# solislemuslab/BayesianNetworkRegression.jl

Measured on NVIDIA B200. Metric: gibbs_iters_per_sec_all_chains, higher is better.
Workload: dtype f64

## Files before the change

bayesiannetworkregression.jl_b200/csrc/bnr_api.cu:

```cuda
#include <chrono>
#include <cstdio>
#include <cstdlib>
#include <cstring>
#include <mutex>
#include <string>
#include <vector>
#include <cuda_runtime.h>
#include <nvtx3/nvToolsExt.h>
#include "../../include/bnr.h"
#include "bnr_engine.cuh"
#include "bnr_kernels.h"

static_assert(BNR_ST_JITTER == BNR_ST_JITTER_ && BNR_ST_SIGMA_NOTPD == BNR_ST_SIGMA_NOTPD_ &&
              BNR_ST_G_NOTPD == BNR_ST_G_NOTPD_ && BNR_ST_GIG_CAP == BNR_ST_GIG_CAP_ &&
              BNR_ST_INJ_EXHAUSTED == BNR_ST_INJ_EXHAUSTED_ && BNR_ST_NAN == BNR_ST_NAN_ &&
              BNR_ST_PSI_NOTPD == BNR_ST_PSI_NOTPD_, "status bits out of sync");
static_assert(BNR_COND_THETA == BNR_COND_THETA_ && BNR_COND_DELTA == BNR_COND_DELTA_ && BNR_COND_M == BNR_COND_M_ &&
              BNR_COND_MU == BNR_COND_MU_ && BNR_COND_LAMBDA == BNR_COND_LAMBDA_ && BNR_COND_PI == BNR_COND_PI_,
              "conditional ids out of sync");
static_assert(BNR_MAX_R == bnr::MAX_R, "MAX_R out of sync");

using namespace bnr;

static thread_local std::string g_err;
// ... 20 lines not shown
  int c0 = 0;
  cudaStream_t stream = nullptr;
  cudaGraph_t graph[2] = {nullptr, nullptr};
  cudaGraphExec_t gexec[2] = {nullptr, nullptr};
  cudaEvent_t done = nullptr;
  ForkJoin fj;
  double* ws = nullptr;
  long long* counters = nullptr;
  long long* mom_window = nullptr;
};
constexpr int MAX_GROUPS = 8;

namespace {
struct CacheBlock { void* p; size_t bytes; int device; };
std::mutex g_cache_mu;
std::vector<CacheBlock> g_cache;
size_t g_cache_bytes = 0;
size_t g_cache_limit = (size_t)4 << 30;

void* cache_take(int device, size_t bytes, size_t* got) {
  std::lock_guard<std::mutex> lk(g_cache_mu);
  size_t best = g_cache.size();
  for (size_t i = 0; i < g_cache.size(); ++i)
    if (g_cache[i].device == device && g_cache[i].bytes >= bytes && g_cache[i].bytes <= bytes + bytes / 4 + ((size_t)1 << 20) &&
        (best == g_cache.size() || g_cache[i].bytes < g_cache[best].bytes))
      best = i;
  if (best == g_cache.size()) return nullptr;
  void* p = g_cache[best].p;
  *got = g_cache[best].bytes;
  g_cache_bytes -= g_cache[best].bytes;
  g_cache[best] = g_cache.back();
  g_cache.pop_back();
  return p;
}
void cache_give(int device, void* p, size_t bytes) {
  {
    std::lock_guard<std::mutex> lk(g_cache_mu);
    if (g_cache_bytes + bytes <= g_cache_limit) {
      g_cache.push_back({p, bytes, device});
      g_cache_bytes += bytes;
      return;
    }
  }
  cudaFree(p);
}
}

struct bnr_handle {
  bnr_params p;
  Engine e;
  cudaStream_t stream = nullptr;
  ChainGroup groups[MAX_GROUPS];
  int n_groups = 0;
  bool graphs_ready[2] = {false, false};
  const double* u_first = nullptr;
  cudaEvent_t ev_fork = nullptr;
  ForkJoin fj;
  cudaEvent_t ev0 = nullptr, ev1 = nullptr;
  std::vector<std::pair<void*, size_t>> allocs;
  double* ws = nullptr;
  double* d_inj = nullptr;
  long long inj_len = 0;
  bool aux_on = false;
  Aux aux_saved = {};
  long long win[5] = {0, 0, 0, 1, 0};
  long long blk_len = 0;
  long long mom_half = 0;
  long long launches = 0;
  long long graph_kernels = 0;
  bool xg_valid = false;
  bool ran = false;
  double* d_rhat = nullptr;
  double* d_tmp = nullptr;
  size_t tmp_doubles = 0;
  double* d_acov = nullptr;
  double* d_cmean = nullptr;
  int ess_lag = -1;
  long long ess_rows = 0;
  size_t acov_cap = 0;
  long long* d_esswin = nullptr;
  double* ess_stream_buf = nullptr;
  size_t ess_stream_cap = 0;
  long long ess_stream_N = 0;
};

static int raw_alloc(bnr_handle* h, void** out, size_t bytes) {
  size_t got = bytes;
  void* p = cache_take(h->p.device, bytes, &got);
  if (!p) { CK(cudaMalloc(&p, bytes)); got = bytes; }
  h->allocs.push_back({p, got});
  *out = p;
  return 0;
}

static void release_alloc(bnr_handle* h, void* p) {
  if (!p) return;
  for (size_t i = 0; i < h->allocs.size(); ++i)
    if (h->allocs[i].first == p) {
      cache_give(h->p.device, p, h->allocs[i].second);
      h->allocs[i] = h->allocs.back();
      h->allocs.pop_back();
      return;
    }
}

struct Scratch {
  int device; void* p = nullptr; size_t bytes = 0;
  Scratch(int dev, size_t b) : device(dev), bytes((b + 255) / 256 * 256) {
    size_t got = bytes;
    p = cache_take(device, bytes, &got);
    if (p) bytes = got;
    else if (cudaMalloc(&p, bytes) != cudaSuccess) p = nullptr;
  }
  ~Scratch() { if (p) cache_give(device, p, bytes); }
};

template <typename T>
static int dalloc(bnr_handle* h, T** ptr, size_t count, bool zero = true) {
  void* p = nullptr;
  const size_t bytes = count * sizeof(T) + 16;
  int r = raw_alloc(h, &p, bytes);
  if (r) return r;
  if (zero) CK(cudaMemsetAsync(p, 0, bytes, h->stream));
  *ptr = (T*)p;
  return 0;
}
static int alloc_table(bnr_handle* h, RowTable& t, bool nan_fill, const char* what) {
  if (int r = dalloc(h, &t.base, t.doubles(), false)) {
    cudaGetLastError();
    return fail(r, std::string(what) + " (" + std::to_string(8.0 * (double)t.doubles()) + " bytes): " + g_err);
  }
  if (nan_fill) CK(cudaMemsetAsync(t.base, 0xff, sizeof(double) * t.doubles(), h->stream));
  return BNR_OK;
}
#define DA(ptr, count)                          \
  do {                                          \
    int _r = dalloc(h, &(ptr), (count));        \
    if (_r) return _r;                          \
  } while (0)

extern "C" int bnr_version(void) { return BNR_VERSION; }
extern "C" const char* bnr_last_error(void) { return g_err.c_str(); }

extern "C" void bnr_default_params(bnr_params* p) {
  memset(p, 0, sizeof(*p));
  p->num_chains = 2;
  p->eta = 1.01; p->zeta = 1.0; p->iota = 1.0; p->a_delta = 1.0; p->b_delta = 1.0; p->nu = 10.0;
  p->trace_full_chains = 1; p->trace_gamma_xi_all = 1; p->gig_inject_len = 64;
}

static int var_size(const Dims& d, int var) {
  switch (var) {
    case BNR_VAR_TAU2: case BNR_VAR_THETA: case BNR_VAR_DELTA: case BNR_VAR_MU: return 1;
    case BNR_VAR_U: return d.R * d.V;
    case BNR_VAR_XI: return d.V;
    case BNR_VAR_GAMMA: case BNR_VAR_S: return d.q;
    case BNR_VAR_M: return d.R * d.R;
    case BNR_VAR_LAMBDA: return d.R;
    case BNR_VAR_PI: return 3 * d.R;
  }
  return -1;
}
static int row_offset(const Dims& d, int var) {
  const int R = d.R, V = d.V, q = d.q;
  const int o[BNR_NUM_VARS] = {0, 1, 1 + V * R, 1 + V * R + V, 1 + V * R + V + q, 1 + V * R + V + 2 * q,
                               2 + V * R + V + 2 * q, 3 + V * R + V + 2 * q, 3 + V * R + V + 2 * q + R * R,
                               4 + V * R + V + 2 * q + R * R, 4 + V * R + V + 2 * q + R * R + R};
  return o[var];
}

static int create_fork_join(ForkJoin& f, int panels, int side_prio, int hi_prio) {
  CK(cudaStreamCreateWithPriority(&f.side, cudaStreamNonBlocking, side_prio));
  CK(cudaStreamCreateWithPriority(&f.side_hi, cudaStreamNonBlocking, hi_prio));
  CK(cudaEventCreateWithFlags(&f.fork, cudaEventDisableTiming));
  CK(cudaEventCreateWithFlags(&f.join, cudaEventDisableTiming));
  f.npool = 4 * panels;
  f.pool = new cudaEvent_t[f.npool]();
  for (int i = 0; i < f.npool; ++i) CK(cudaEventCreateWithFlags(&f.pool[i], cudaEventDisableTiming));
  return BNR_OK;
}

static void destroy_fork_join(ForkJoin& f) {
  if (f.side) cudaStreamDestroy(f.side);
  if (f.side_hi) cudaStreamDestroy(f.side_hi);
  if (f.fork) cudaEventDestroy(f.fork);
  if (f.join) cudaEventDestroy(f.join);
  for (int i = 0; i < f.npool && f.pool; ++i)
    if (f.pool[i]) cudaEventDestroy(f.pool[i]);
  delete[] f.pool;
  f = ForkJoin();
}

static int create_impl(bnr_handle* h, const bnr_params* p, const double* X, const double* y);

extern "C" int bnr_create(const bnr_params* p, const double* X, const double* y, bnr_handle** out) {
  if (!p || !X || !y || !out) return fail(BNR_EINVAL, "null argument");
  if (p->n < 1 || p->V < 2 || p->R < 1 || p->R > BNR_MAX_R || p->num_chains < 1)
    return fail(BNR_EINVAL, "need n >= 1, V >= 2, 1 <= R <= 16, num_chains >= 1");
  if (!(p->nu > p->R - 1)) return fail(BNR_EINVAL, "nu must exceed R - 1 (InverseWishart degrees of freedom)");
  int ndev = 0;
  if (cudaGetDeviceCount(&ndev) != cudaSuccess || ndev == 0)
    return fail(BNR_ENODEV, "no CUDA device visible: libbnr has no CPU fallback");
  if (p->device < 0 || p->device >= ndev) return fail(BNR_EINVAL, "device ordinal out of range");
  CK(cudaSetDevice(p->device));
  int cc_major = 0;
  CK(cudaDeviceGetAttribute(&cc_major, cudaDevAttrComputeCapabilityMajor, p->device));
  if (cc_major < 10) return fail(BNR_ENODEV, "libbnr is built for sm_100a (B200) only");

  bnr_handle* h = new bnr_handle();
  h->p = *p;
  const double t0 = wall_ms();
  const int rc = create_impl(h, p, X, y);
  if (g_timing) fprintf(stderr, "[bnr] bnr_create %.2f ms (%zu device buffers)\n", wall_ms() - t0, h->allocs.size());
  if (rc != BNR_OK) {
    const std::string msg = g_err;
    bnr_destroy(h);
    g_err = msg;
    return rc;
  }
  *out = h;
  return BNR_OK;
}

static int create_impl(bnr_handle* h, const bnr_params* p, const double* X, const double* y) {
  if (h->p.gig_inject_len <= 0) h->p.gig_inject_len = 64;
  Dims& d = h->e.d;
  d.n = p->n; d.V = p->V; d.R = p->R; d.C = p->num_chains; d.C_total = p->num_chains;
  d.q = p->V * (p->V + 1) / 2;
  d.np = (p->n + 1 + TILE_N - 1) / TILE_N * TILE_N;
  d.qp = (d.q + TILE_K - 1) / TILE_K * TILE_K;
  {
    const double qd = d.q, nd = d.n;
    const double cost_q = qd * qd * qd / 3.0 + 4.0 * qd * qd, cost_n = nd * nd * qd + nd * nd * nd / 3.0;
    const int qp128 = (d.q + 1 + TILE_N - 1) / TILE_N * TILE_N;
    const int small = bwd_stream_max_dim(), large = chol_max_dim();
    int mode = p->gamma_mode;
    if (mode != BNR_GAMMA_NFORM && mode != BNR_GAMMA_QFORM) {
      mode = (cost_q < cost_n && qp128 <= small) ? BNR_GAMMA_QFORM : BNR_GAMMA_NFORM;
      if ((mode == BNR_GAMMA_QFORM ? qp128 : d.np) > small) {
        const bool q_fits = qp128 <= large, n_fits = d.np <= large;
        mode = (q_fits && (cost_q < cost_n || !n_fits)) ? BNR_GAMMA_QFORM : BNR_GAMMA_NFORM;
      }
    }
    d.gmode = mode;
    if (mode == BNR_GAMMA_QFORM) d.qp = qp128;
    d.gdim = mode == BNR_GAMMA_QFORM ? d.qp : d.np;
  }
  d.nparts = (d.q + PART_BLOCK - 1) / PART_BLOCK;
  d.chain_offset = p->chain_offset;
  d.chain_offset_local = 0;
  d.gigK = h->p.gig_inject_len;
  d.seed = p->seed;
  d.eta = p->eta; d.zeta = p->zeta; d.iota = p->iota; d.a_delta = p->a_delta; d.b_delta = p->b_delta; d.nu = p->nu;
  const size_t need = sizeof(double) * ((size_t)d.V * d.R + 2 * d.R * d.R + 2 + 4 * (2 * d.V + 2 * d.R * d.R + 3 * d.R));
  if (need > 200 * 1024 || d.gdim > chol_max_dim()) {
    return fail(BNR_EINVAL, "problem too large for the per-chain shared-memory kernels (V*R > 200 KB of shared memory, or factored dimension > 32768: n <= 32767 in the n-form, V <= 255 in the q-form)");
  }
  CK(cudaStreamCreateWithFlags(&h->stream, cudaStreamNonBlocking));
  CK(cudaEventCreate(&h->ev0));
  CK(cudaEventCreate(&h->ev1));
  linalg_setup();
  {
    const int clusters = bwd_cluster_capacity(d.gdim);
    if (clusters < 0) return fail(BNR_ECUDA, "cudaOccupancyMaxActiveClusters failed for the cluster back solve");
    if (clusters == 0)
      return fail(BNR_ECUDA, "this device cannot co-schedule the back solve's cluster of 8 CTAs with ~210 KB of shared memory each (factored dimension > 8192)");
  }
  if (!tmap_setup()) return fail(BNR_ECUDA, "cuTensorMapEncodeTiled is not available from this driver (TMA tensor maps are required)");
  small_kernels_setup();

  Engine& e = h->e;
  const size_t C = d.C;
  const double t_create0 = wall_ms();
  double *dX, *dy;
  DA(dX, (size_t)d.qp * d.np);
  DA(dy, (size_t)d.np);
  CK(cudaMemcpy2DAsync(dX, (size_t)d.np * sizeof(double), X, (size_t)d.n * sizeof(double),
                       (size_t)d.n * sizeof(double), (size_t)d.q, cudaMemcpyHostToDevice, h->stream));
  CK(cudaMemcpyAsync(dy, y, (size_t)d.n * sizeof(double), cudaMemcpyHostToDevice, h->stream));
  e.X = dX; e.y = dy;
  if (g_timing) { cudaStreamSynchronize(h->stream); fprintf(stderr, "[bnr]   X, y upload done at +%.2f ms\n", wall_ms() - t_create0); }
  std::vector<int2> lk(d.q);
  {
    int j = 0;
    for (int k = 0; k < d.V; ++k)
      for (int l = k; l < d.V; ++l) lk[j++] = make_int2(l, k);
  }
  int2* dlk;
  DA(dlk, (size_t)d.q);
  CK(cudaMemcpyAsync(dlk, lk.data(), sizeof(int2) * d.q, cudaMemcpyHostToDevice, h->stream));
  CK(cudaStreamSynchronize(h->stream));
  e.edge_lk = dlk;

  DA(e.tau2, C); DA(e.u, C * d.V * d.R); DA(e.u_alt, C * d.V * d.R); DA(e.xi, C * d.V);
  h->u_first = e.u;
  DA(e.gamma, C * d.qp); DA(e.S, C * d.qp); DA(e.theta, C); DA(e.Delta, C); DA(e.M, C * d.R * d.R);
  DA(e.mu, C); DA(e.lambda, C * d.R); DA(e.pi, C * 3 * d.R);
  DA(e.W, C * d.qp); DA(e.v, C * d.qp); DA(e.t, C * d.qp);
  DA(e.xg, C * d.np); DA(e.xv, C * d.np); DA(e.rhs, C * d.np);
  DA(e.G, C * d.gdim * d.gdim + 2048);
  DA(e.Linv, C * (size_t)(d.gdim / TILE_N) * TILE_N * TILE_N);
  CK(cudaMemsetAsync(e.Linv, 0, sizeof(double) * C * (size_t)(d.gdim / TILE_N) * TILE_N * TILE_N, h->stream));
  e.syrk_ws = nullptr; e.syrk_ws_cap = 0;
  e.gram_planes = nullptr; e.gram_rscale = nullptr;
  if (gram_i8_selected(d)) {
    DA(e.gram_planes, C * gram_i8_plane_bytes(d));
    DA(e.gram_rscale, C * d.np);
  } else if (d.gmode == BNR_GAMMA_NFORM) {
    const int smax = syrk_splits(d, d.C);
    if (smax > 1) {
      e.syrk_ws_cap = smax - 1;
      DA(e.syrk_ws, C * (size_t)e.syrk_ws_cap * d.gdim * d.gdim);
    }
  }
  e.XtX = nullptr;
  if (d.gmode == BNR_GAMMA_QFORM) {
    std::vector<double> xt((size_t)d.np * d.qp, 0.0), ones((size_t)d.np, 1.0);
    for (int j = 0; j < d.q; ++j)
      for (int i = 0; i < d.n; ++i) xt[(size_t)i * d.qp + j] = X[(size_t)i + (size_t)d.n * j];
    double *dXT = nullptr, *dOnes = nullptr, *dXtX = nullptr;
    DA(dXT, xt.size());
    DA(dOnes, ones.size());
    DA(dXtX, (size_t)d.qp * d.qp);
    CK(cudaMemcpyAsync(dXT, xt.data(), xt.size() * sizeof(double), cudaMemcpyHostToDevice, h->stream));
    CK(cudaMemcpyAsync(dOnes, ones.data(), ones.size() * sizeof(double), cudaMemcpyHostToDevice, h->stream));
    launch_xtx(d, dXT, dOnes, dXtX, h->stream);
    CK(cudaStreamSynchronize(h->stream));
    release_alloc(h, dXT);
    release_alloc(h, dOnes);
    e.XtX = dXtX;
  }
  DA(e.partials, C * d.nparts * (2 * MAX_R + 1));
  DA(e.tau2_part, C * 2 * TAU2_MAX_BLOCKS);
  DA(e.tau2_ticket, C);
  DA(e.status, C);
  DA(e.iter, 1); DA(e.trace_row, 1);
  DA(e.moments, C * 2 * (d.V + d.q) * 2);
  DA(e.mom_window, 5);
  e.bmom = nullptr; e.bmom_nb = 0;
  e.ess_ring = e.ess_head = e.ess_acc = e.ess_sum = nullptr; e.ess_win = nullptr; e.ess_L = e.ess_cap = 0;
  DA(h->d_esswin, 4);
  DA(h->ws, x_times_workspace_doubles(d));
  DA(h->d_rhat, (size_t)(d.V + d.q));
  const long long trace_rows = p->trace_rows > 0 ? p->trace_rows : 0;
  e.tr_full = {nullptr, trace_rows, 4 + d.V * d.R + d.V + 2 * d.q + d.R * d.R + d.R + 3 * d.R, 0};
  e.tr_gx = {nullptr, trace_rows, d.V + d.q, 0};
  if (trace_rows > 0) {
    e.tr_full.chains = p->trace_full_chains < 0 ? 0 : (p->trace_full_chains < d.C ? p->trace_full_chains : d.C);
    if (p->trace_gamma_xi_all) e.tr_gx.chains = d.C;
    else if (p->trace_gamma_xi_chains > 0) e.tr_gx.chains = p->trace_gamma_xi_chains < d.C ? p->trace_gamma_xi_chains : d.C;
  }
  if (e.tr_full.chains > 0) if (int r = alloc_table(h, e.tr_full, false, "full-state trace")) return r;
  if (e.tr_gx.chains > 0) if (int r = alloc_table(h, e.tr_gx, false, "gamma/xi trace")) return r;
  {
    int ng_auto = d.C >= 6 ? 3 : (d.C >= 4 ? 4 : (d.C >= 2 ? 2 : 1));
    if (d.gmode == BNR_GAMMA_NFORM && d.C >= 4 && syrk_splits(d, d.C) > 1) ng_auto = 2;
    if (d.gmode == BNR_GAMMA_QFORM && d.C >= 2 && d.C < 24) ng_auto = 2;
    if (gram_i8_selected(d) && d.C < 12) ng_auto = 1;
    int ng = p->chain_groups > 0 ? p->chain_groups : ng_auto;
    if (ng > MAX_GROUPS) ng = MAX_GROUPS;
    if (ng > d.C) ng = d.C;
    h->n_groups = ng;
    CK(cudaEventCreateWithFlags(&h->ev_fork, cudaEventDisableTiming));
    const int panels = d.gdim / TILE_N;
    if (int r = create_fork_join(h->fj, panels, 0, 0)) return r;
    int plo = 0, phi = 0;
    CK(cudaDeviceGetStreamPriorityRange(&plo, &phi));
    for (int g = 0; g < ng; ++g) {
      ChainGroup& G = h->groups[g];
      CK(cudaStreamCreateWithPriority(&G.stream, cudaStreamNonBlocking, phi));
      CK(cudaEventCreateWithFlags(&G.done, cudaEventDisableTiming));
      if (int r = create_fork_join(G.fj, panels, plo, phi)) return r;
      DA(G.ws, x_times_workspace_doubles(d));
      DA(G.counters, 2);
      DA(G.mom_window, 5);
    }
  }
  if (g_timing) { cudaStreamSynchronize(h->stream); fprintf(stderr, "[bnr]   buffers, streams, events at +%.2f ms\n", wall_ms() - t_create0); }
  h->tmp_doubles = (size_t)1 << 22;
  DA(h->d_tmp, h->tmp_doubles);
  e.inj = nullptr; e.inj_stride = 0;
  memset(&e.aux, 0, sizeof(e.aux));
  CK(cudaStreamSynchronize(h->stream));
  if (!tmaps_check(e)) return fail(BNR_ECUDA, "cuTensorMapEncodeTiled refused a tensor map of this problem's geometry");
  return BNR_OK;
}

static void drop_graph(bnr_handle* h);

extern "C" int bnr_trim_cache(void) {
  std::vector<CacheBlock> blocks;
  {
    std::lock_guard<std::mutex> lk(g_cache_mu);
    blocks.swap(g_cache);
    g_cache_bytes = 0;
  }
  int cur = 0;
  cudaGetDevice(&cur);
  for (auto& b : blocks) { cudaSetDevice(b.device); cudaFree(b.p); }
  cudaSetDevice(cur);
  return BNR_OK;
}

extern "C" int bnr_set_cache_limit(int64_t bytes) {
  if (bytes < 0) return fail(BNR_EINVAL, "negative limit");
  { std::lock_guard<std::mutex> lk(g_cache_mu); g_cache_limit = (size_t)bytes; }
  if (bytes == 0) return bnr_trim_cache();
  return BNR_OK;
}

extern "C" int bnr_destroy(bnr_handle* h) {
  if (!h) return BNR_OK;
  const double t_destroy0 = wall_ms();
  cudaSetDevice(h->p.device);
  if (h->stream) cudaStreamSynchronize(h->stream);
  drop_graph(h);
  for (int g = 0; g < h->n_groups; ++g) {
    if (h->groups[g].stream) { cudaStreamSynchronize(h->groups[g].stream); cudaStreamDestroy(h->groups[g].stream); }
    if (h->groups[g].done) cudaEventDestroy(h->groups[g].done);
    destroy_fork_join(h->groups[g].fj);
  }
  destroy_fork_join(h->fj);
  if (h->ev_fork) cudaEventDestroy(h->ev_fork);
  for (auto& a : h->allocs) cache_give(h->p.device, a.first, a.second);
  if (h->ev0) cudaEventDestroy(h->ev0);
  if (h->ev1) cudaEventDestroy(h->ev1);
  if (h->stream) cudaStreamDestroy(h->stream);
  delete h;
  if (g_timing) fprintf(stderr, "[bnr] bnr_destroy %.2f ms\n", wall_ms() - t_destroy0);
  return BNR_OK;
}

static void drop_graph(bnr_handle* h) {
  for (int g = 0; g < h->n_groups; ++g) {
    ChainGroup& G = h->groups[g];
    for (int par = 0; par < 2; ++par) {
      if (G.gexec[par]) { cudaGraphExecDestroy(G.gexec[par]); G.gexec[par] = nullptr; }
      if (G.graph[par]) { cudaGraphDestroy(G.graph[par]); G.graph[par] = nullptr; }
    }
  }
  h->graphs_ready[0] = h->graphs_ready[1] = false;
}

static void refresh_xg(bnr_handle* h) {
  launch_x_times(h->e, 0, h->e.gamma, h->e.xg, h->ws, h->stream);
  h->xg_valid = true;
}

static void mark(cudaEvent_t* marks, int k, cudaStream_t s) {
  if (marks) cudaEventRecord(marks[k], s);
}

static void run_gamma(Engine& e, double* ws, const ForkJoin& fj, cudaStream_t s, int gig_flags, bool syrk_forked = false,
                      cudaEvent_t* marks = nullptr) {
  if (e.d.gmode == BNR_GAMMA_QFORM) {
    launch_edge_prep(e, 2, s);
    launch_x_times(e, 0, e.W, e.xv, ws, s);
    launch_rhs(e, s);
    launch_x_times(e, 1, e.rhs, e.t, ws, s);
    mark(marks, 3, s);
    launch_build_P(e, s);
    mark(marks, 4, s);
    launch_cholesky(e, e.t, fj, s);
    mark(marks, 5, s);
    launch_chol_solve(e, e.t, e.v, s);
    mark(marks, 6, s);
    launch_gamma_gig(e, (gig_flags & ~1) | ((gig_flags & 1) ? 4 : 0), s);
    return;
  }
  launch_edge_prep(e, 1, s);
  launch_x_times(e, 0, e.v, e.xv, ws, s);
  launch_rhs(e, s);
  mark(marks, 3, s);
  if (syrk_forked) cudaStreamWaitEvent(s, fj.join, 0);
  else launch_syrk_G(e, s);
  mark(marks, 4, s);
  launch_cholesky(e, e.rhs, fj, s);
  mark(marks, 5, s);
  launch_chol_solve(e, e.rhs, nullptr, s);
  mark(marks, 6, s);
  launch_x_times(e, 1, e.rhs, e.t, ws, s);
  launch_gamma_gig(e, gig_flags, s);
}

static void enqueue_record(Engine& e, double* ws, const ForkJoin& fj, cudaStream_t s, bool sweep_done, bool pred_forked,
                           bool xg_stale) {
  launch_record(e, sweep_done, s);
  if (sweep_done && e.ess_ring) launch_ess_stream(e, s);
  if (e.pred.base) {
    if (pred_forked) cudaStreamWaitEvent(s, fj.join, 0);
    else launch_pred_product(e, s);
    launch_pred_record(e, sweep_done, s);
  }
  if (e.ll.base) {
    if (xg_stale) launch_x_times(e, 0, e.gamma, e.xg, ws, s);
    launch_loglik_record(e, s);
  }
  launch_advance(e, sweep_done, s);
}

static void enqueue_sweep(Engine& e, double* ws, const ForkJoin& fj, cudaStream_t s, cudaEvent_t* marks = nullptr) {
  NvtxRange sweep("bnr sweep");
  mark(marks, 0, s);
  const bool fork_syrk = !marks && e.d.gmode == BNR_GAMMA_NFORM && !e.aux.G_copy;
  if (fork_syrk) {
    NvtxRange r("gamma: G = X D X' + I (forked)");
    cudaEventRecord(fj.fork, s);
    cudaStreamWaitEvent(fj.side, fj.fork, 0);
    launch_syrk_G(e, fj.side);
    cudaEventRecord(fj.join, fj.side);
  }
  { NvtxRange r("tau2"); launch_tau2(e, s); }
  mark(marks, 1, s);
  { NvtxRange r("u, xi"); launch_uxi(e, s); }
  std::swap(e.u, e.u_alt);
  mark(marks, 2, s);
  { NvtxRange r("gamma + D (GIG)"); run_gamma(e, ws, fj, s, 3, fork_syrk, marks); }
  mark(marks, 7, s);
  const bool fork_pred = !marks && e.pred.base;
  if (fork_pred) {
    NvtxRange r("predictions: X_new gamma");
    cudaEventRecord(fj.fork, s);
    cudaStreamWaitEvent(fj.side, fj.fork, 0);
    launch_pred_product(e, fj.side);
    cudaEventRecord(fj.join, fj.side);
  }
  {
    NvtxRange r("theta, Delta, M, mu, Lambda, pi");
    launch_x_times(e, 0, e.gamma, e.xg, ws, s);
    launch_finish(e, (1 << BNR_COND_THETA) | (1 << BNR_COND_DELTA) | (1 << BNR_COND_M) | (1 << BNR_COND_MU) |
                         (1 << BNR_COND_LAMBDA) | (1 << BNR_COND_PI), s);
  }
  NvtxRange r("record");
  enqueue_record(e, ws, fj, s, true, fork_pred, false);
  mark(marks, 8, s);
}

static Engine group_view(const bnr_handle* h, int c0, int Cg, long long* counters, long long* mom_window) {
  Engine v = h->e;
  const Dims& d = h->e.d;
  const size_t c = (size_t)c0;
  v.d.C = Cg;
  v.d.chain_offset = d.chain_offset + c0;
  v.d.chain_offset_local = c0;
  v.tau2 += c; v.theta += c; v.Delta += c; v.mu += c; v.status += c;
  v.u += c * d.V * d.R; v.u_alt += c * d.V * d.R; v.xi += c * d.V;
  v.gamma += c * d.qp; v.S += c * d.qp; v.W += c * d.qp; v.v += c * d.qp; v.t += c * d.qp;
  v.M += c * d.R * d.R; v.lambda += c * d.R; v.pi += c * 3 * d.R;
  v.xg += c * d.np; v.xv += c * d.np; v.rhs += c * d.np;
  v.G += c * d.gdim * d.gdim; if (v.syrk_ws) v.syrk_ws += c * (size_t)v.syrk_ws_cap * d.gdim * d.gdim; v.Linv += c * (size_t)(d.gdim / TILE_N) * TILE_N * TILE_N;
  if (v.gram_planes) { v.gram_planes += c * gram_i8_plane_bytes(d); v.gram_rscale += c * d.np; }
  v.partials += c * d.nparts * (2 * MAX_R + 1);
  v.moments += c * 2 * (d.V + d.q) * 2;
  if (v.bmom) v.bmom += c * (size_t)v.bmom_nb * (d.V + d.q) * 2;
  if (v.ess_ring) {
    const size_t P = (size_t)d.V + d.q;
    v.ess_ring += c * (size_t)v.ess_cap * P; v.ess_head += c * (size_t)v.ess_L * P;
    v.ess_acc += c * (size_t)(v.ess_L + 1) * P; v.ess_sum += c * 2 * P;
  }
  v.tr_full = v.tr_full.view(c0, Cg); v.tr_gx = v.tr_gx.view(c0, Cg);
  v.pred = v.pred.view(c0, Cg); v.ll = v.ll.view(c0, Cg);
  if (v.pred_ws) v.pred_ws += c * (size_t)v.pred_splits * v.pred_mp;
  v.iter = counters; v.trace_row = counters + 1; v.mom_window = mom_window;
  v.inj = nullptr; v.inj_stride = 0;
  memset(&v.aux, 0, sizeof(v.aux));
  return v;
}

static int build_graphs(bnr_handle* h) {
  const int par = (h->e.u != h->u_first) ? 1 : 0;
  if (h->graphs_ready[par]) return BNR_OK;
  const double t0 = wall_ms();
  const long long before = g_launches;
  const int C = h->e.d.C, ng = h->n_groups;
  for (int g = 0; g < ng; ++g) {
    ChainGroup& G = h->groups[g];
    const int c0 = (int)((long long)C * g / ng), c1 = (int)((long long)C * (g + 1) / ng);
    G.c0 = c0;
    G.e = group_view(h, c0, c1 - c0, G.counters, G.mom_window);
    Engine e = G.e;
    CK(cudaStreamBeginCapture(G.stream, cudaStreamCaptureModeThreadLocal));
    enqueue_sweep(e, G.ws, G.fj, G.stream);
    enqueue_sweep(e, G.ws, G.fj, G.stream);
    CK(cudaStreamEndCapture(G.stream, &G.graph[par]));
    CK(cudaGraphInstantiate(&G.gexec[par], G.graph[par], cudaGraphInstantiateFlagUseNodePriority));
  }
  h->graph_kernels = g_launches - before;
  h->graphs_ready[par] = true;
  if (g_timing) fprintf(stderr, "[bnr] graph capture + instantiate (%d groups, %lld kernels) %.2f ms\n", ng, h->graph_kernels, wall_ms() - t0);
  return BNR_OK;
}

extern "C" int bnr_init_state(bnr_handle* h) {
  if (!h) return fail(BNR_EINVAL, "null handle");
  CK(cudaSetDevice(h->p.device));
  Engine& e = h->e;
  CK(cudaMemsetAsync(e.iter, 0, sizeof(long long), h->stream));
  CK(cudaMemsetAsync(e.trace_row, 0, sizeof(long long), h->stream));
  CK(cudaMemsetAsync(e.status, 0, sizeof(int) * e.d.C, h->stream));
  launch_init(e, h->stream);
  enqueue_record(e, h->ws, h->fj, h->stream, false, false, true);
  h->xg_valid = false;
  CK(cudaGetLastError());
  CK(cudaStreamSynchronize(h->stream));
  return BNR_OK;
}

extern "C" int bnr_run(bnr_handle* h, int64_t n_iters) {
  if (!h || n_iters < 0) return fail(BNR_EINVAL, "bad arguments");
  NvtxRange range("bnr_run");
  CK(cudaSetDevice(h->p.device));
  CK(cudaEventRecord(h->ev0, h->stream));
  if (!h->xg_valid) { const long long b0 = g_launches; refresh_xg(h); h->launches += g_launches - b0; }
  int64_t left = n_iters;
  if (h->e.inj == nullptr && !h->aux_on && left >= 2) {
    int r = build_graphs(h);
    if (r) return r;
    const int par = (h->e.u != h->u_first) ? 1 : 0;
    CK(cudaEventRecord(h->ev_fork, h->stream));
    for (int g = 0; g < h->n_groups; ++g) {
      ChainGroup& G = h->groups[g];
      CK(cudaStreamWaitEvent(G.stream, h->ev_fork, 0));
      CK(cudaMemcpyAsync(G.counters, h->e.iter, sizeof(long long), cudaMemcpyDeviceToDevice, G.stream));
      CK(cudaMemcpyAsync(G.counters + 1, h->e.trace_row, sizeof(long long), cudaMemcpyDeviceToDevice, G.stream));
    }
    for (; left >= 2; left -= 2) {
      for (int g = 0; g < h->n_groups; ++g) CK(cudaGraphLaunch(h->groups[g].gexec[par], h->groups[g].stream));
      h->launches += h->graph_kernels;
    }
    for (int g = 0; g < h->n_groups; ++g) {
      CK(cudaEventRecord(h->groups[g].done, h->groups[g].stream));
      CK(cudaStreamWaitEvent(h->stream, h->groups[g].done, 0));
    }
    CK(cudaMemcpyAsync(h->e.iter, h->groups[0].counters, sizeof(long long), cudaMemcpyDeviceToDevice, h->stream));
    CK(cudaMemcpyAsync(h->e.trace_row, h->groups[0].counters + 1, sizeof(long long), cudaMemcpyDeviceToDevice, h->stream));
  }
  for (; left > 0; --left) {
    const long long before = g_launches;
    enqueue_sweep(h->e, h->ws, h->fj, h->stream);
    h->launches += g_launches - before;
  }
  CK(cudaEventRecord(h->ev1, h->stream));
  if (h->e.inj == nullptr && !h->aux_on && (h->graphs_ready[0] || h->graphs_ready[1])) {
    int r = build_graphs(h);
    if (r) return r;
  }
  CK(cudaGetLastError());
  h->ran = true;
  return BNR_OK;
}

extern "C" int bnr_sync(bnr_handle* h) {
  if (!h) return fail(BNR_EINVAL, "null handle");
  CK(cudaSetDevice(h->p.device));
  CK(cudaStreamSynchronize(h->stream));
  CK(cudaGetLastError());
  return BNR_OK;
}

extern "C" int bnr_last_run_ms(bnr_handle* h, float* ms) {
  if (!h || !ms || !h->ran) return fail(BNR_ESTATE, "no run recorded");
  CK(cudaSetDevice(h->p.device));
  CK(cudaEventSynchronize(h->ev1));
  CK(cudaEventElapsedTime(ms, h->ev0, h->ev1));
  return BNR_OK;
}

extern "C" int bnr_iteration(bnr_handle* h, int64_t* completed) {
  if (!h || !completed) return fail(BNR_EINVAL, "null argument");
  CK(cudaSetDevice(h->p.device));
  long long v = 0;
  CK(cudaMemcpyAsync(&v, h->e.iter, sizeof(v), cudaMemcpyDeviceToHost, h->stream));
  CK(cudaStreamSynchronize(h->stream));
  *completed = v;
  return BNR_OK;
}

extern "C" int bnr_set_trace_row(bnr_handle* h, int64_t row) {
  if (!h || row < 0) return fail(BNR_EINVAL, "bad arguments");
  CK(cudaSetDevice(h->p.device));
  long long v = row;
  CK(cudaMemcpyAsync(h->e.trace_row, &v, sizeof(v), cudaMemcpyHostToDevice, h->stream));
  CK(cudaStreamSynchronize(h->stream));
  return BNR_OK;
}

extern "C" int bnr_get_trace_row(bnr_handle* h, int64_t* row) {
  if (!h || !row) return fail(BNR_EINVAL, "null argument");
  CK(cudaSetDevice(h->p.device));
  long long v = 0;
  CK(cudaMemcpyAsync(&v, h->e.trace_row, sizeof(v), cudaMemcpyDeviceToHost, h->stream));
  CK(cudaStreamSynchronize(h->stream));
  *row = v;
  return BNR_OK;
}

extern "C" int bnr_copy_trace_rows(bnr_handle* h, int64_t dst, int64_t src, int64_t count) {
  if (!h || dst < 0 || src < 0 || count < 0) return fail(BNR_EINVAL, "bad arguments");
  CK(cudaSetDevice(h->p.device));
  Engine& e = h->e;
  const struct { const RowTable& t; const char* range_msg; } all[] = {
      {e.tr_full, "rows out of range"}, {e.tr_gx, "rows out of range"},
      {e.pred, "rows beyond the prediction table"}, {e.ll, "rows beyond the log-likelihood table"}};
  bool any = false;
  int max_row = 0;
  for (const auto& a : all) {
    if (!a.t.base) continue;
    if (dst + count > a.t.rows || src + count > a.t.rows) return fail(BNR_EINVAL, a.range_msg);
    if (a.t.width > max_row) max_row = a.t.width;
    any = true;
  }
  if (!any) return BNR_OK;
  if (count == 0 || dst == src) return BNR_OK;
  const bool overlap = !(dst + count <= src || src + count <= dst);
  Scratch sc(h->p.device, overlap ? (size_t)count * max_row * sizeof(double) : 256);
  if (overlap && !sc.p) return fail(BNR_ENOMEM, "device scratch allocation failed");
  for (const auto& a : all) {
    if (!a.t.base) continue;
    const size_t bytes = (size_t)count * a.t.width * sizeof(double);
    for (int c = 0; c < a.t.chains; ++c) {
      if (!overlap) {
        CK(cudaMemcpyAsync(a.t.row(c, dst), a.t.row(c, src), bytes, cudaMemcpyDeviceToDevice, h->stream));
      } else {
        CK(cudaMemcpyAsync(sc.p, a.t.row(c, src), bytes, cudaMemcpyDeviceToDevice, h->stream));
        CK(cudaMemcpyAsync(a.t.row(c, dst), sc.p, bytes, cudaMemcpyDeviceToDevice, h->stream));
      }
    }
  }
  CK(cudaStreamSynchronize(h->stream));
  return BNR_OK;
}

static int push_windows(bnr_handle* h) {
  CK(cudaMemcpyAsync(h->e.mom_window, h->win, sizeof(h->win), cudaMemcpyHostToDevice, h->stream));
  for (int g = 0; g < h->n_groups; ++g)
    CK(cudaMemcpyAsync(h->groups[g].mom_window, h->win, sizeof(h->win), cudaMemcpyHostToDevice, h->stream));
  CK(cudaStreamSynchronize(h->stream));
  return BNR_OK;
}

extern "C" int bnr_set_moment_window(bnr_handle* h, int64_t first, int64_t len) {
  if (!h || len < 0) return fail(BNR_EINVAL, "bad arguments");
  CK(cudaSetDevice(h->p.device));
  h->win[0] = first; h->win[1] = len;
  int r = push_windows(h);
  if (r) return r;
  h->mom_half = len / 2;
  return BNR_OK;
}

extern "C" int bnr_set_moment_blocks(bnr_handle* h, int64_t first_sweep, int64_t block_len, int32_t nblocks) {
  if (!h || nblocks < 0 || (nblocks > 0 && block_len < 1)) return fail(BNR_EINVAL, "bad arguments");
  CK(cudaSetDevice(h->p.device));
  const Dims& d = h->e.d;
  if (nblocks > h->e.bmom_nb) {
    CK(cudaStreamSynchronize(h->stream));
    drop_graph(h);
    void* p = nullptr;
    release_alloc(h, h->e.bmom);
    h->e.bmom = nullptr; h->e.bmom_nb = 0;
    int r = raw_alloc(h, &p, sizeof(double) * (size_t)d.C * nblocks * (d.V + d.q) * 2);
    if (r) return r;
    h->e.bmom = (double*)p;
    h->e.bmom_nb = nblocks;
  }
  h->win[2] = first_sweep; h->win[3] = block_len > 0 ? block_len : 1; h->win[4] = nblocks;
  h->blk_len = block_len;
  return push_windows(h);
}

__global__ void k_merge_blocks(const double* __restrict__ bmom, int nb_cap, int nparam, int first_block, int per_half,
                               long long blen, double* __restrict__ mom) {
  const int p = blockIdx.x * blockDim.x + threadIdx.x;
  if (p >= nparam) return;
  const int c = blockIdx.y, half = blockIdx.z;
  double n = 0.0, mean = 0.0, m2 = 0.0;
  for (int b = 0; b < per_half; ++b) {
    const double* m = bmom + (((size_t)c * nb_cap + first_block + half * per_half + b) * nparam + p) * 2;
    const double nb_ = (double)blen, delta = m[0] - mean, tot = n + nb_;
    mean += delta * nb_ / tot;
    m2 += m[1] + delta * delta * n * nb_ / tot;
    n = tot;
  }
  double* o = mom + (((size_t)c * 2 + half) * nparam + p) * 2;
  o[0] = mean; o[1] = m2;
}

extern "C" int bnr_moments_from_blocks(bnr_handle* h, int32_t first_block, int32_t nblocks) {
  if (!h || first_block < 0 || nblocks < 2 || (nblocks & 1)) return fail(BNR_EINVAL, "need an even number of blocks >= 2");
  CK(cudaSetDevice(h->p.device));
  if (!h->e.bmom || first_block + nblocks > (int)h->win[4]) return fail(BNR_ESTATE, "blocks not configured (bnr_set_moment_blocks)");
  const Dims& d = h->e.d;
  const int np_ = d.V + d.q;
  dim3 grid((np_ + 127) / 128, d.C, 2);
  k_merge_blocks<<<grid, 128, 0, h->stream>>>(h->e.bmom, h->e.bmom_nb, np_, first_block, nblocks / 2, h->blk_len, h->e.moments);
  CK(cudaGetLastError());
  CK(cudaStreamSynchronize(h->stream));
  h->mom_half = (long long)(nblocks / 2) * h->blk_len;
  return BNR_OK;
}

extern "C" int bnr_moments_device(bnr_handle* h, double** dev_ptr, int64_t* count) {
  if (!h || !dev_ptr || !count) return fail(BNR_EINVAL, "null argument");
  CK(cudaSetDevice(h->p.device));
  CK(cudaStreamSynchronize(h->stream));
  *dev_ptr = h->e.moments;
  *count = (int64_t)h->e.d.C * 2 * (h->e.d.V + h->e.d.q) * 2;
  return BNR_OK;
}

extern "C" int bnr_rhat_from_moments(int device, const double* dev_moments, int32_t total_chains, int32_t V,
                                     int32_t q, int64_t half_len, double* rhat_xi, double* rhat_gamma) {
  if (!dev_moments || total_chains < 1 || half_len < 2) return fail(BNR_EINVAL, "bad arguments (need half_len >= 2)");
  CK(cudaSetDevice(device));
  Scratch sc(device, sizeof(double) * (V + q));
  if (!sc.p) return fail(BNR_ENOMEM, "device scratch allocation failed");
  double* d_out = (double*)sc.p;
  launch_rhat(dev_moments, total_chains, V + q, half_len, d_out, 0);
  std::vector<double> host(V + q);
  CK(cudaMemcpy(host.data(), d_out, sizeof(double) * (V + q), cudaMemcpyDeviceToHost));
  if (rhat_xi) memcpy(rhat_xi, host.data(), sizeof(double) * V);
  if (rhat_gamma) memcpy(rhat_gamma, host.data() + V, sizeof(double) * q);
  return BNR_OK;
}

__global__ void k_moments_from_trace(RowTable tr, long long first, long long nrows, double* __restrict__ mom) {
  const int nparam = tr.width, p = blockIdx.x * blockDim.x + threadIdx.x;
  if (p >= nparam) return;
  const int c = blockIdx.y, half = blockIdx.z;
  const long long h = nrows / 2;
  const long long r0 = first + (half == 0 ? 0 : nrows - h);
  const double* __restrict__ base = tr.row(c, r0) + p;
  double s = 0.0;
  for (long long r = 0; r < h; ++r) s += base[(size_t)r * nparam];
  const double mean = s / (double)h;
  double m2 = 0.0;
  for (long long r = 0; r < h; ++r) { const double dl = base[(size_t)r * nparam] - mean; m2 += dl * dl; }
  double* m = mom + (((size_t)c * 2 + half) * nparam + p) * 2;
  m[0] = mean; m[1] = m2;
}

extern "C" int bnr_moments_from_trace(bnr_handle* h, int64_t first_row, int64_t nrows) {
  if (!h || first_row < 0 || nrows < 0) return fail(BNR_EINVAL, "bad arguments");
  CK(cudaSetDevice(h->p.device));
  Engine& e = h->e;
  if (!e.tr_gx.base || e.tr_gx.chains < e.d.C)
    return fail(BNR_ESTATE, "gamma/xi traces of every chain are needed (trace_gamma_xi_all = 0): use the streaming "
                            "moments of bnr_set_moment_window instead");
  if (first_row + nrows > e.tr_gx.rows) return fail(BNR_EINVAL, "rows beyond trace capacity");
  if (nrows / 2 < 2) return fail(BNR_EINVAL, "need at least 4 rows");
  dim3 grid((e.tr_gx.width + 127) / 128, e.d.C, 2);
  k_moments_from_trace<<<grid, 128, 0, h->stream>>>(e.tr_gx, first_row, nrows, e.moments);
  CK(cudaGetLastError());
  CK(cudaStreamSynchronize(h->stream));
  h->mom_half = nrows / 2;
  return BNR_OK;
}

extern "C" int bnr_moment_half_len(bnr_handle* h, int64_t* half_len) {
  if (!h || !half_len) return fail(BNR_EINVAL, "null argument");
  CK(cudaSetDevice(h->p.device));
  *half_len = h->mom_half;
  return BNR_OK;
}

extern "C" int bnr_rhat(bnr_handle* h, double* rhat_xi, double* rhat_gamma) {
  if (!h) return fail(BNR_EINVAL, "null handle");
  CK(cudaSetDevice(h->p.device));
  if (h->mom_half < 2) return fail(BNR_ESTATE, "moment window too short for R-hat");
  const Dims& d = h->e.d;
  launch_rhat(h->e.moments, d.C, d.V + d.q, h->mom_half, h->d_rhat, h->stream);
  std::vector<double> host(d.V + d.q);
  CK(cudaMemcpyAsync(host.data(), h->d_rhat, sizeof(double) * (d.V + d.q), cudaMemcpyDeviceToHost, h->stream));
  CK(cudaStreamSynchronize(h->stream));
  if (rhat_xi) memcpy(rhat_xi, host.data(), sizeof(double) * d.V);
  if (rhat_gamma) memcpy(rhat_gamma, host.data() + d.V, sizeof(double) * d.q);
  return BNR_OK;
}

extern "C" int bnr_var_size(bnr_handle* h, int32_t var, int64_t* n) {
  if (!h || !n || var < 0 || var >= BNR_NUM_VARS) return fail(BNR_EINVAL, "bad arguments");
  CK(cudaSetDevice(h->p.device));
// ... 738 lines not shown
```

bayesiannetworkregression.jl_b200/csrc/bnr_engine.cuh:

```cuda
#pragma once
#include <cstdint>
#include <cuda_runtime.h>
#include "bnr_rng.cuh"

namespace bnr {

constexpr int MAX_R = 16;
constexpr int TILE_N = 128;
constexpr int TILE_K = 16;
constexpr int TAU2_MAX_BLOCKS = 32;
constexpr int PART_BLOCK = 256;

struct Dims {
  int n, V, R, q, C;
  int C_total;
  int np, qp;
  int gmode;
  int gdim;
  int nparts;
  int chain_offset;
  int chain_offset_local;
  int gigK;
  uint64_t seed;
  double eta, zeta, iota, a_delta, b_delta, nu;
};

struct InjLayout {
  int64_t tau2, uxi, z1, z2, S, theta, Delta, M, mu, lambda, pi, total;
  __host__ __device__ static InjLayout make(int n, int V, int R, int K) {
    InjLayout l;
    const int64_t q = (int64_t)V * (V + 1) / 2;
    int64_t o = 0;
    l.tau2 = o; o += 1;
    l.uxi = o; o += (int64_t)V * (R + 1);
    l.z1 = o; o += q;
    l.z2 = o; o += n;
    l.S = o; o += q * K;
    l.theta = o; o += 1;
    l.Delta = o; o += 3;
    l.M = o; o += R + R * (R - 1) / 2;
    l.mu = o; o += 1;
    l.lambda = o; o += R;
    l.pi = o; o += 3 * R;
    l.total = o;
    return l;
  }
};

struct InitLayout {
  int64_t S, pi, lambda, xi, M, u, gamma, total;
  __host__ __device__ static InitLayout make(int V, int R) {
    InitLayout l;
    const int64_t q = (int64_t)V * (V + 1) / 2;
    int64_t o = 0;
    l.S = o; o += q;
    l.pi = o; o += 3 * R;
    l.lambda = o; o += R;
    l.xi = o; o += V;
    l.M = o; o += R + R * (R - 1) / 2;
    l.u = o; o += (int64_t)V * R;
    l.gamma = o; o += q;
    l.total = o;
    return l;
  }
};

struct Aux {
  double* tau2_params;
  double* sigma_inv;
  double* sigma_chol;
  double* mu_t;
  double* log_odds;
  double* chi;
  double* theta_params;
  double* delta_params;
  double* m_params;
  double* mu_params;
  double* lambda_logw;
  double* lambda_w;
  double* pi_alpha;
  double* gig_used;
  double* G_copy;
};

struct RowTable {
  double* base; long long rows; int width; int chains;
  __host__ __device__ bool holds(int c, long long r) const { return base && c < chains && r < rows; }
  __host__ __device__ double* row(int c, long long r) const { return base + ((size_t)c * rows + r) * width; }
  RowTable view(int c0, int Cg) const {
    RowTable v = *this;
    v.chains = chains - c0 < 0 ? 0 : (chains - c0 > Cg ? Cg : chains - c0);
    v.base = base && v.chains > 0 ? row(c0, 0) : nullptr;
    return v;
  }
  size_t doubles() const { return (size_t)chains * rows * width; }
};

struct Engine {
  Dims d;
  const double* X;
  const double* y;
  const int2* edge_lk;
  const double* XtX;
  double* tau2; double* u; double* u_alt; double* xi; double* gamma; double* S; double* theta;
  double* Delta; double* M; double* mu; double* lambda; double* pi;
  double* W;
  double* v;
  double* t;
  double* xg;
  double* xv;
  double* rhs;
  double* G;
  double* syrk_ws;
  int syrk_ws_cap;
  signed char* gram_planes;
  double* gram_rscale;
  double* Linv;
  double* partials;
  double* tau2_part;
  unsigned* tau2_ticket;
  int* status;
  long long* iter;
  long long* trace_row;
  double* moments;
  long long* mom_window;
  double* bmom;
  int bmom_nb;
  double* ess_ring;
  double* ess_head;
  double* ess_acc;
  double* ess_sum;
  const long long* ess_win;
  int ess_L, ess_cap;
  RowTable tr_full;
  RowTable tr_gx;
  RowTable pred;
  const double* Xp;
  int pred_mp, pred_mode, pred_splits;
  double* pred_ws;
  RowTable ll;
  const double* inj;
  long long inj_stride;
  Aux aux;
};

__device__ __forceinline__ RngKey chain_key(const Dims& d, int c) {
  return make_key(d.seed, (uint32_t)(d.chain_offset + c));
}

}
```

bayesiannetworkregression.jl_b200/csrc/bnr_kernels.h:

```cpp
#pragma once
#include <cuda_runtime.h>
#include "bnr_engine.cuh"

#define BNR_ST_JITTER_ 1
#define BNR_ST_SIGMA_NOTPD_ 2
#define BNR_ST_G_NOTPD_ 4
#define BNR_ST_GIG_CAP_ 8
#define BNR_ST_INJ_EXHAUSTED_ 16
#define BNR_ST_NAN_ 32
#define BNR_ST_PSI_NOTPD_ 64
#define BNR_COND_THETA_ 4
#define BNR_COND_DELTA_ 5
#define BNR_COND_M_ 6
#define BNR_COND_MU_ 7
#define BNR_COND_LAMBDA_ 8
#define BNR_COND_PI_ 9

namespace bnr {

extern thread_local long long g_launches;

void launch_tau2(const Engine& e, cudaStream_t s);
void launch_uxi(const Engine& e, cudaStream_t s);
void launch_edge_prep(const Engine& e, int draw_v, cudaStream_t s);
void launch_rhs(const Engine& e, cudaStream_t s);
void launch_gamma_gig(const Engine& e, int flags, cudaStream_t s);
void launch_finish(const Engine& e, int mask, cudaStream_t s);
void launch_init(const Engine& e, cudaStream_t s);
void launch_record(const Engine& e, int sweep_done, cudaStream_t s);
void launch_advance(const Engine& e, int inc_iter, cudaStream_t s);
void launch_rhat(const double* mom, int chains, int nparams, long long h, double* out, cudaStream_t s);
void launch_test_chol_jitter(int R, const double* Ain, double* Aused, double* Lout, int* status, cudaStream_t s);
void launch_rng_dump(const Dims& d, int chain, long long iteration, int site, int element, int kind, double shape,
                     int count, double* out, cudaStream_t s);

void launch_x_times(const Engine& e, int trans, const double* in, double* out, double* splitk_ws, cudaStream_t s);
void launch_x_times(const Dims& d, int trans, const double* A, int lda, int M, int K, const double* in, double* out,
                    double* splitk_ws, cudaStream_t s);
size_t x_times_workspace_doubles(const Dims& d);
int pred_splits(const Dims& d, int mp);
void launch_pred_product(const Engine& e, cudaStream_t s);
void launch_pred_record(const Engine& e, int sweep_done, cudaStream_t s);
void launch_loglik_record(const Engine& e, cudaStream_t s);
void launch_syrk_G(const Engine& e, cudaStream_t s);
int syrk_splits(const Dims& d, int C);
constexpr int GRAM_I8_QP_MIN = 1024;
constexpr int GRAM_I8_QP_MAX = 18724;
bool gram_i8_selected(const Dims& d);
size_t gram_i8_plane_bytes(const Dims& d);
struct ForkJoin {
  cudaStream_t side = nullptr;
  cudaStream_t side_hi = nullptr;
  cudaEvent_t fork = nullptr, join = nullptr;
  cudaEvent_t* pool = nullptr;
  int npool = 0;
};
void launch_cholesky(const Engine& e, double* rhs, const ForkJoin& fj, cudaStream_t s);
void launch_chol_solve(const Engine& e, double* rhs, const double* addz, cudaStream_t s);
void launch_xtx(const Dims& d, const double* XT, const double* ones, double* XtX, cudaStream_t s);
void launch_build_P(const Engine& e, cudaStream_t s);
int chol_max_dim();
int bwd_stream_max_dim();
int bwd_cluster_capacity(int N);
bool tmaps_check(const Engine& e);
bool tmap_setup();
void linalg_setup();
void small_kernels_setup();

void launch_summary_select(const double* rows, size_t rowlen, int off, int nelem, long long first, long long count,
                           long long rank_lo, long long rank_hi, double* mean_out, double* lo_out, double* hi_out,
                           cudaStream_t s);
void launch_chain_mean(const RowTable& tr, long long first, long long N, double* cmean, cudaStream_t s);
void launch_acov_sum(const RowTable& tr, long long first, long long N, int L, const double* cmean, double* acov,
                     cudaStream_t s);
void launch_ess_stream(const Engine& e, cudaStream_t s);
void launch_ess_stream_finalize(const Engine& e, long long N, double* acov, double* cmean, cudaStream_t s);
size_t pred_select_ws_bytes(long long N, int m);
void launch_pred_select(const double* rows, long long N, int m, long long rank_lo, long long rank_hi, double* mean,
                        double* lo, double* hi, void* ws, cudaStream_t s);
long long loo_tail_len(long long N);
long long loo_tail_max();
size_t loo_ws_bytes(long long N, int n);
void launch_loo(const double* rows, long long N, int n, double* out, void* ws, cudaStream_t s);
void launch_ess_finish(const double* acov_parts, int nparts, const double* cmeans, int chains, int P, long long N,
                       int L, double* ess, double* lag_used, cudaStream_t s);

}
```

bayesiannetworkregression.jl_b200/csrc/bnr_linalg.cu:

```cuda
#include <cstdio>
#include <cstdlib>
#include <cstring>
#include <cuda.h>
#include "bnr_engine.cuh"
#include "bnr_kernels.h"

namespace bnr {

__device__ __forceinline__ void dmma884(double& c0, double& c1, double a, double b) {
  asm volatile("mma.sync.aligned.m8n8k4.row.col.f64.f64.f64.f64 {%0,%1}, {%2}, {%3}, {%0,%1};\n"
               : "+d"(c0), "+d"(c1) : "d"(a), "d"(b));
}
__device__ __forceinline__ double neg_bits(double x) {
  return __longlong_as_double(__double_as_longlong(x) ^ (long long)0x8000000000000000ull);
}
__device__ __forceinline__ void cp_async_commit() { asm volatile("cp.async.commit_group;\n" ::); }
template <int N>
__device__ __forceinline__ void cp_async_wait() { asm volatile("cp.async.wait_group %0;\n" ::"n"(N)); }
__device__ __forceinline__ void cp_async16(void* smem, const void* gmem) {
  const unsigned sa = (unsigned)__cvta_generic_to_shared(smem);
  asm volatile("cp.async.cg.shared.global [%0], [%1], 16;\n" ::"r"(sa), "l"(gmem));
}

__device__ __forceinline__ unsigned smem_u32(const void* p) { return (unsigned)__cvta_generic_to_shared(p); }
// ... 1070 lines not shown
    for (int s = 0; s < nstages; ++s) { mbar_init(&full[s], 1); mbar_init(&empty[s], 8); }
    for (int s = 0; s < BWC_SLOTS; ++s) mbar_init(&sfull[s], 8 * (BWC_K - 1));
    for (int i = 0; i < BWC_K * BWC_SLOTS; ++i) mbar_init(&sfree[i], 1);
    asm volatile("fence.mbarrier_init.release.cluster;\n" ::: "memory");
  }
  __syncthreads();
  cluster_sync_all();

  if (warp == 8) {
    if (lane == 0) {
      int p = 0;
      for (int J = T - 1; J >= 0; --J) {
        const int Ilast = (J % BWC_K == r) ? J : J + 1;
        for (int I = Itop; I >= Ilast; I -= BWC_K) {
          for (int h = 0; h < BW_NH; ++h, ++p) {
            const int stage = p % nstages;
            mbar_wait(&empty[stage], ((p / nstages) & 1) ^ 1);
            mbar_expect_tx(&full[stage], BW_STAGE_DBL * 8u);
            double* dst = ring + (size_t)stage * BW_STAGE_DBL;
            if (I == J) tma_load_2d(dst, &tmL, 0, (c * T + J) * PB + h * BW_COLS, &full[stage]);
            else tma_load_2d(dst, &tmG, I * PB, c * N + J * PB + h * BW_COLS, &full[stage]);
          }
        }
      }
    }
  } else {
    const double unscale = out[(size_t)c * out_stride + m];
    for (int id = tid; id < nown * PB; id += 256) {
      const int I = r + BWC_K * (id / PB), k = I * PB + id % PB;
      xo[id] = (I < T && k < m) ? Gc[(size_t)k * N + m] * unscale + (addz ? addz[(size_t)c * addz_stride + k] : 0.0) : 0.0;
    }
    named_bar_sync(1, 256);

    int it = 0;
    for (int J = T - 1; J >= 0; --J) {
      const int o = J % BWC_K, u = (T - 1 - J) / BWC_K;
      const int s = u % BWC_SLOTS;
      const unsigned par = (u / BWC_SLOTS) & 1;
      double pr[BW_NH][BW_CPW];
#pragma unroll
      for (int h = 0; h < BW_NH; ++h)
#pragma unroll
        for (int q = 0; q < BW_CPW; ++q) pr[h][q] = 0.0;
      for (int I = Itop; I > J; I -= BWC_K) {
        const double* v = xo + (size_t)(I / BWC_K) * PB;
        const double v0 = v[lane], v1 = v[lane + 32], v2 = v[lane + 64], v3 = v[lane + 96];
#pragma unroll
        for (int h = 0; h < BW_NH; ++h, ++it) {
          const int stage = it % nstages;
          mbar_wait(&full[stage], (it / nstages) & 1);
          const double* B = ring + (size_t)stage * BW_STAGE_DBL + (size_t)(warp * BW_CPW) * PB + lane;
          double acc[BW_CPW];
#pragma unroll
          for (int q = 0; q < BW_CPW; ++q)
            acc[q] = B[q * PB] * v0 + B[q * PB + 32] * v1 + B[q * PB + 64] * v2 + B[q * PB + 96] * v3;
#pragma unroll
          for (int q = 0; q < BW_CPW; ++q) {
#pragma unroll
            for (int o2 = 16; o2 > 0; o2 >>= 1) acc[q] += __shfl_xor_sync(0xffffffffu, acc[q], o2);
            pr[h][q] += acc[q];
          }
          __syncwarp();
          if (lane == 0) mbar_arrive(&empty[stage]);
        }
      }
      if (o != r) {
        if (lane == 0) {
          mbar_wait_cluster(&sfree[o * BWC_SLOTS + s], par ^ 1);
          const unsigned dst = mapa_rank(slot + ((size_t)s * BWC_K + r) * PB, (unsigned)o);
#pragma unroll
          for (int h = 0; h < BW_NH; ++h)
#pragma unroll
            for (int q = 0; q < BW_CPW; ++q) st_cluster_f64(dst + 8u * (h * BW_COLS + warp * BW_CPW + q), pr[h][q]);
          mbar_arrive_remote(mapa_rank(&sfull[s], (unsigned)o));
        }
        __syncwarp();
        continue;
      }
      double* bJ = xo + (size_t)(J / BWC_K) * PB;
      if (lane == 0) {
        mbar_wait_cluster(&sfull[s], par);
        const double* sl = slot + (size_t)s * BWC_K * PB;
#pragma unroll
        for (int h = 0; h < BW_NH; ++h)
#pragma unroll
          for (int q = 0; q < BW_CPW; ++q) {
            const int col = h * BW_COLS + warp * BW_CPW + q;
            double t = bJ[col];
#pragma unroll
            for (int rr = 0; rr < BWC_K; ++rr) t -= (rr == r) ? pr[h][q] : sl[rr * PB + col];
            bJ[col] = t;
          }
      }
      __syncwarp();
      named_bar_sync(1, 256);
      if (tid == 0) {
        for (int rr = 0; rr < BWC_K; ++rr)
          if (rr != r) mbar_arrive_remote(mapa_rank(&sfree[r * BWC_SLOTS + s], (unsigned)rr));
      }
      const double v0 = bJ[lane], v1 = bJ[lane + 32], v2 = bJ[lane + 64], v3 = bJ[lane + 96];
      double xn[BW_NH][BW_CPW];
#pragma unroll
      for (int h = 0; h < BW_NH; ++h, ++it) {
        const int stage = it % nstages;
        mbar_wait(&full[stage], (it / nstages) & 1);
        const double* B = ring + (size_t)stage * BW_STAGE_DBL + (size_t)(warp * BW_CPW) * PB + lane;
        double acc[BW_CPW];
#pragma unroll
        for (int q = 0; q < BW_CPW; ++q)
          acc[q] = B[q * PB] * v0 + B[q * PB + 32] * v1 + B[q * PB + 64] * v2 + B[q * PB + 96] * v3;
#pragma unroll
        for (int q = 0; q < BW_CPW; ++q) {
#pragma unroll
          for (int o2 = 16; o2 > 0; o2 >>= 1) acc[q] += __shfl_xor_sync(0xffffffffu, acc[q], o2);
          xn[h][q] = acc[q];
        }
        __syncwarp();
        if (lane == 0) mbar_arrive(&empty[stage]);
      }
      named_bar_sync(1, 256);
      if (lane == 0) {
#pragma unroll
        for (int h = 0; h < BW_NH; ++h)
#pragma unroll
          for (int q = 0; q < BW_CPW; ++q) bJ[h * BW_COLS + warp * BW_CPW + q] = xn[h][q];
      }
      __syncwarp();
      named_bar_sync(1, 256);
    }
    for (int id = tid; id < nown * PB; id += 256) {
      const int I = r + BWC_K * (id / PB);
      if (I < T) out[(size_t)c * out_stride + (size_t)I * PB + id % PB] = xo[id];
    }
  }
  cluster_sync_all();
}

__global__ void k_copy_sym(const double* __restrict__ G, size_t chain_stride, int np, double* __restrict__ out) {
  const int c = blockIdx.y, j = blockIdx.x;
  const double* Gc = G + (size_t)c * chain_stride;
  double* o = out + (size_t)c * np * np;
  for (int i = threadIdx.x; i < np; i += blockDim.x) {
    const double v = (i >= j) ? Gc[(size_t)j * np + i] : Gc[(size_t)i * np + j];
    o[(size_t)j * np + i] = v;
  }
}

constexpr int XM_BM = 128, XM_BN = 64, XM_BK = 16, XM_STAGES = 3;
constexpr int XM_LDM = 132, XM_LDK = 20;
constexpr int XM_A_DBL = (XM_BK * XM_LDM > XM_BM * XM_LDK) ? XM_BK * XM_LDM : XM_BM * XM_LDK;
constexpr int XM_STAGE_DBL = XM_A_DBL + XM_BN * XM_LDK;
constexpr size_t XMMA_SMEM = sizeof(double) * XM_STAGES * XM_STAGE_DBL;

__device__ __forceinline__ void cp_async16_zfill(void* smem, const void* gmem, bool valid) {
  const unsigned sa = (unsigned)__cvta_generic_to_shared(smem);
  const int sz = valid ? 16 : 0;
  asm volatile("cp.async.cg.shared.global [%0], [%1], 16, %2;\n" ::"r"(sa), "l"(gmem), "r"(sz));
}

template <int TRANS>
__global__ void __launch_bounds__(256) k_xmma(const double* __restrict__ X, int np, int M, int K, int N,
                                              const double* __restrict__ in, int ldin, double* __restrict__ out,
                                              int ldout, int k_per_split) {
  extern __shared__ __align__(16) double sm[];
  const int tid = threadIdx.x, lane = tid & 31, warp = tid >> 5;
  const int lk = lane & 3, lr = lane >> 2, wm = warp & 3, wn = warp >> 2;
  const int m0 = blockIdx.x * XM_BM, n0 = blockIdx.y * XM_BN;
  const int kbeg = blockIdx.z * k_per_split;
  const int kend = min(K, kbeg + k_per_split);
  const int nsteps = (kend - kbeg + XM_BK - 1) / XM_BK;
  double* o = out + (size_t)blockIdx.z * N * ldout;

  auto load_stage = [&](int step) {
    double* As = sm + (size_t)(step % XM_STAGES) * XM_STAGE_DBL;
    double* Vs = As + XM_A_DBL;
    const int k0 = kbeg + step * XM_BK;
    if (TRANS == 0) {
#pragma unroll
      for (int r = 0; r < 4; ++r) {
        const int id = tid + 256 * r, kk = id >> 6, mm = (id & 63) * 2;
        cp_async16_zfill(As + kk * XM_LDM + mm, X + (size_t)(k0 + kk) * np + m0 + mm, m0 + mm < M);
      }
    } else {
#pragma unroll
      for (int r = 0; r < 4; ++r) {
        const int id = tid + 256 * r, mm = id >> 3, kk = (id & 7) * 2;
        const bool ok = m0 + mm < M;
        cp_async16_zfill(As + mm * XM_LDK + kk, X + (size_t)(ok ? m0 + mm : 0) * np + k0 + kk, ok);
      }
    }
#pragma unroll
    for (int r = 0; r < 2; ++r) {
      const int id = tid + 256 * r, nn = id >> 3, kk = (id & 7) * 2;
      const bool ok = n0 + nn < N;
      cp_async16_zfill(Vs + nn * XM_LDK + kk, in + (size_t)(ok ? n0 + nn : 0) * ldin + k0 + kk, ok);
    }
  };

  double acc[4][4][2];
#pragma unroll
  for (int a = 0; a < 4; ++a)
#pragma unroll
    for (int b = 0; b < 4; ++b) acc[a][b][0] = acc[a][b][1] = 0.0;
  int nfv = (N - n0 - wn * 32 + 7) >> 3;
  nfv = nfv < 0 ? 0 : (nfv > 4 ? 4 : nfv);

  for (int s = 0; s < XM_STAGES - 1; ++s) {
    if (s < nsteps) load_stage(s);
    cp_async_commit();
  }
  for (int step = 0; step < nsteps; ++step) {
    cp_async_wait<XM_STAGES - 2>();
    __syncthreads();
    if (step + XM_STAGES - 1 < nsteps) load_stage(step + XM_STAGES - 1);
    cp_async_commit();
    const double* As = sm + (size_t)(step % XM_STAGES) * XM_STAGE_DBL;
    const double* Vs = As + XM_A_DBL;
    if (nfv == 0) continue;
#pragma unroll
    for (int k4 = 0; k4 < XM_BK / 4; ++k4) {
      const int kr = k4 * 4 + lk;
      double af[4], bf[4];
#pragma unroll
      for (int mf = 0; mf < 4; ++mf)
        af[mf] = (TRANS == 0) ? As[kr * XM_LDM + wm * 32 + mf * 8 + lr] : As[(wm * 32 + mf * 8 + lr) * XM_LDK + kr];
#pragma unroll
      for (int nf = 0; nf < 4; ++nf) bf[nf] = (nf < nfv) ? Vs[(wn * 32 + nf * 8 + lr) * XM_LDK + kr] : 0.0;
#pragma unroll
      for (int nf = 0; nf < 4; ++nf) {
        if (nf < nfv) {
#pragma unroll
          for (int mf = 0; mf < 4; ++mf) dmma884(acc[mf][nf][0], acc[mf][nf][1], af[mf], bf[nf]);
        }
      }
    }
  }
  cp_async_wait<0>();
#pragma unroll
  for (int mf = 0; mf < 4; ++mf) {
    const int mm = m0 + wm * 32 + mf * 8 + lr;
#pragma unroll
    for (int nf = 0; nf < 4; ++nf) {
      const int nn = n0 + wn * 32 + nf * 8 + 2 * lk;
      if (mm < M) {
        if (nn < N) o[(size_t)nn * ldout + mm] = acc[mf][nf][0];
        if (nn + 1 < N) o[(size_t)(nn + 1) * ldout + mm] = acc[mf][nf][1];
      }
    }
  }
}

__global__ void k_splitk_reduce(const double* __restrict__ ws, double* __restrict__ out, size_t count, int splits) {
  const size_t i = (size_t)blockIdx.x * blockDim.x + threadIdx.x;
  if (i >= count) return;
  double s = 0.0;
  for (int z = 0; z < splits; ++z) s += ws[(size_t)z * count + i];
  out[i] = s;
}

static int x_times_splits(int M, int K, int C_total) {
  const int tiles = ((M + XM_BM - 1) / XM_BM) * ((C_total + XM_BN - 1) / XM_BN);
  int ks = (2 * 148 + tiles - 1) / tiles;
  const int kmax = K / (4 * XM_BK) > 0 ? K / (4 * XM_BK) : 1;
  if (ks > kmax) ks = kmax;
  if (ks > 64) ks = 64;
  if (ks < 1) ks = 1;
  return ks;
}

size_t x_times_workspace_doubles(const Dims& d) {
  const int a = x_times_splits(d.np, d.qp, d.C_total), b = x_times_splits(d.qp, d.np, d.C_total);
  const size_t wa = (size_t)a * d.C_total * d.np, wb = (size_t)b * d.C_total * d.qp;
  return wa > wb ? wa : wb;
}

int pred_splits(const Dims& d, int mp) { return x_times_splits(mp, d.qp, d.C_total); }

void launch_x_times(const Dims& d, int trans, const double* A, int lda, int M, int K, const double* in, double* out,
                    double* ws, cudaStream_t s) {
  const int N = d.C, ldin = K, ldout = M;
  const int ks = x_times_splits(M, K, d.C_total);
  const int kper = ((K + ks - 1) / ks + XM_BK - 1) / XM_BK * XM_BK;
  dim3 grid((M + XM_BM - 1) / XM_BM, (N + XM_BN - 1) / XM_BN, ks);
  double* dst = (ks == 1 && out) ? out : ws;
  ++g_launches;
  if (trans) k_xmma<1><<<grid, 256, XMMA_SMEM, s>>>(A, lda, M, K, N, in, ldin, dst, ldout, kper);
  else k_xmma<0><<<grid, 256, XMMA_SMEM, s>>>(A, lda, M, K, N, in, ldin, dst, ldout, kper);
  if (ks > 1 && out) {
    const size_t count = (size_t)N * ldout;
    ++g_launches; k_splitk_reduce<<<(unsigned)((count + 255) / 256), 256, 0, s>>>(ws, out, count, ks);
  }
}

void launch_x_times(const Engine& e, int trans, const double* in, double* out, double* ws, cudaStream_t s) {
  const Dims& d = e.d;
  launch_x_times(d, trans, e.X, d.np, trans ? d.qp : d.np, trans ? d.np : d.qp, in, out, ws, s);
}

void launch_pred_product(const Engine& e, cudaStream_t s) {
  launch_x_times(e.d, 0, e.Xp, e.pred_mp, e.pred_mp, e.d.qp, e.gamma, nullptr, e.pred_ws, s);
}

__global__ void k_gram_i8(const __grid_constant__ CUtensorMap tmA, const __grid_constant__ CUtensorMap tmB,
                          const double* __restrict__ rscale, double* __restrict__ G, int np, int nvalid, int nkb);
extern const size_t GI_SMEM_BYTES;

void linalg_setup() {
  cudaFuncSetAttribute(k_xmma<0>, cudaFuncAttributeMaxDynamicSharedMemorySize, (int)XMMA_SMEM);
  cudaFuncSetAttribute(k_xmma<1>, cudaFuncAttributeMaxDynamicSharedMemorySize, (int)XMMA_SMEM);
  cudaFuncSetAttribute(k_gram_syrk, cudaFuncAttributeMaxDynamicSharedMemorySize, (int)SYRK_SMEM);
  cudaFuncSetAttribute(k_gram_i8, cudaFuncAttributeMaxDynamicSharedMemorySize, (int)GI_SMEM_BYTES);
  cudaFuncSetAttribute(k_chol_update, cudaFuncAttributeMaxDynamicSharedMemorySize, (int)SYRK_SMEM);
  cudaFuncSetAttribute(k_trsm_dmma, cudaFuncAttributeMaxDynamicSharedMemorySize, (int)SYRK_SMEM);
  cudaFuncSetAttribute(k_potf2_inv, cudaFuncAttributeMaxDynamicSharedMemorySize, (int)POTF2_SMEM);
  cudaFuncSetAttribute(k_bwd_stream, cudaFuncAttributeMaxDynamicSharedMemorySize, 227 * 1024);
  cudaFuncSetAttribute(k_bwd_cluster, cudaFuncAttributeMaxDynamicSharedMemorySize, 227 * 1024);
  cudaFuncSetAttribute(k_small_tile<1, 4>, cudaFuncAttributeMaxDynamicSharedMemorySize, (int)small_tile_smem(32));
  cudaFuncSetAttribute(k_small_tile<2, 4>, cudaFuncAttributeMaxDynamicSharedMemorySize, (int)small_tile_smem(32));
  cudaFuncSetAttribute(k_small_tile<1, 2>, cudaFuncAttributeMaxDynamicSharedMemorySize, (int)small_tile_smem(16));
  cudaFuncSetAttribute(k_small_tile<2, 2>, cudaFuncAttributeMaxDynamicSharedMemorySize, (int)small_tile_smem(16));
  cudaFuncSetAttribute(k_small_tile<1, 8>, cudaFuncAttributeMaxDynamicSharedMemorySize, (int)small_tile_smem(64));
  cudaFuncSetAttribute(k_small_tile<2, 8>, cudaFuncAttributeMaxDynamicSharedMemorySize, (int)small_tile_smem(64));
}

typedef CUresult (*TmapEncodeFn)(CUtensorMap*, CUtensorMapDataType, cuuint32_t, void*, const cuuint64_t*, const cuuint64_t*,
                                 const cuuint32_t*, const cuuint32_t*, CUtensorMapInterleave, CUtensorMapSwizzle,
                                 CUtensorMapL2promotion, CUtensorMapFloatOOBfill);
static TmapEncodeFn g_tmap_encode = nullptr;
bool tmap_setup() {
  if (g_tmap_encode) return true;
  void* fn = nullptr;
  cudaDriverEntryPointQueryResult qr;
  if (cudaGetDriverEntryPoint("cuTensorMapEncodeTiled", &fn, cudaEnableDefault, &qr) != cudaSuccess ||
      qr != cudaDriverEntryPointSuccess || !fn)
    return false;
  g_tmap_encode = (TmapEncodeFn)fn;
  return true;
}
static CUresult encode_map(CUtensorMap* m, const double* base, uint64_t rows, uint64_t krows, uint64_t ld, uint32_t box_rows,
                           uint32_t box_k) {
  memset(m, 0, sizeof(*m));
  const cuuint64_t dims[2] = {rows, krows};
  const cuuint64_t strides[1] = {ld * sizeof(double)};
  const cuuint32_t box[2] = {box_rows, box_k};
  const cuuint32_t estr[2] = {1, 1};
  if (!tmap_setup()) return CUDA_ERROR_NOT_SUPPORTED;
  return g_tmap_encode(m, CU_TENSOR_MAP_DATA_TYPE_FLOAT64, 2, const_cast<double*>(base), dims, strides, box, estr,
                       CU_TENSOR_MAP_INTERLEAVE_NONE, CU_TENSOR_MAP_SWIZZLE_NONE, CU_TENSOR_MAP_L2_PROMOTION_L2_256B,
                       CU_TENSOR_MAP_FLOAT_OOB_FILL_NONE);
}
static CUtensorMap make_map(const double* base, uint64_t rows, uint64_t krows, uint64_t ld, uint32_t box_rows,
                            uint32_t box_k = SY_BK) {
  CUtensorMap m;
  const CUresult r = encode_map(&m, base, rows, krows, ld, box_rows, box_k);
  if (r != CUDA_SUCCESS) {
    fprintf(stderr, "[bnr] cuTensorMapEncodeTiled failed (%d) for a %llu x %llu operand, box %u x %d\n", (int)r,
            (unsigned long long)rows, (unsigned long long)krows, box_rows, (int)box_k);
    abort();
  }
  return m;
}
bool tmaps_check(const Engine& e) {
  const Dims& d = e.d;
  const uint64_t N = d.gdim, C = d.C, T = d.gdim / SY_BT;
  CUtensorMap m;
  bool ok = true;
  if (d.gmode != 2) ok = ok && encode_map(&m, e.X, d.np, d.qp, d.np, SY_LDS, SY_BK) == CUDA_SUCCESS;
  for (uint32_t box : {(uint32_t)SY_LDS, (uint32_t)(SY_BT / 2 + 4), (uint32_t)(SY_BT / 4 + 4)})
    ok = ok && encode_map(&m, e.G, N, N * C, N, box, SY_BK) == CUDA_SUCCESS;
  ok = ok && encode_map(&m, e.Linv, SY_BT, SY_BT * T * C, SY_BT, SY_LDS, SY_BK) == CUDA_SUCCESS;
  ok = ok && encode_map(&m, e.G, N, N * C, N, SY_BT, BW_COLS) == CUDA_SUCCESS;
  ok = ok && encode_map(&m, e.Linv, SY_BT, SY_BT * T * C, SY_BT, SY_BT, BW_COLS) == CUDA_SUCCESS;
  return ok;
}

int syrk_splits(const Dims& d, int C) {
  const int T = d.np / SY_BT, tiles = T * (T + 1) / 2, nk = d.qp / SY_BK;
  if (tiles * C >= 148) return 1;
  int s = (4 * 148 + tiles * C - 1) / (tiles * C);
  if (s > nk / 24) s = nk / 24;
  if (s > SYRK_MAX_SPLITS) s = SYRK_MAX_SPLITS;
  return s < 1 ? 1 : s;
}

#ifndef BNR_GI_BK
#define BNR_GI_BK 64
#endif
#ifndef BNR_GI_STAGES
#define BNR_GI_STAGES 2
#endif
constexpr int GI_S = 7;
constexpr int GI_BM = 128, GI_BN = 64;
constexpr int GI_BK = BNR_GI_BK;
constexpr int GI_STAGES = BNR_GI_STAGES;
constexpr int GI_A_PLANE = GI_BM * GI_BK, GI_B_PLANE = GI_BN * GI_BK;
constexpr int GI_STAGE_BYTES = GI_S * (GI_A_PLANE + GI_B_PLANE);
constexpr size_t GI_SMEM = (size_t)GI_STAGES * GI_STAGE_BYTES + 1024 + 256;
const size_t GI_SMEM_BYTES = GI_SMEM;
constexpr int GI_THREADS = 192;
static_assert(GI_BK == 32 || GI_BK == 64 || GI_BK == 128, "k-block = swizzle width");
static_assert(GI_S * GI_BN <= 512, "accumulators exceed tensor memory");

__device__ __forceinline__ unsigned long long gi_desc(unsigned saddr) {
  constexpr unsigned long long layout = GI_BK == 128 ? 2ull : (GI_BK == 64 ? 4ull : 6ull);
  return (unsigned long long)((saddr & 0x3FFFF) >> 4) | (1ull << 16) | ((unsigned long long)((GI_BK * 8) >> 4) << 32) |
         (1ull << 46) | (layout << 61);
}
__host__ __device__ constexpr unsigned gi_idesc(int n) {
  return (2u << 4) | (1u << 7) | (1u << 10) | ((unsigned)(n >> 3) << 17) | ((unsigned)(GI_BM >> 4) << 24);
}

__device__ __forceinline__ void tma_load_3d(void* smem_dst, const CUtensorMap* tm, int x, int y, int z, unsigned long long* bar) {
  asm volatile("cp.async.bulk.tensor.3d.shared::cluster.global.tile.mbarrier::complete_tx::bytes [%0], [%1, {%2, %3, %4}], [%5];\n" ::"r"(
                   smem_u32(smem_dst)), "l"((unsigned long long)tm), "r"(x), "r"(y), "r"(z), "r"(smem_u32(bar)) : "memory");
}
__device__ __forceinline__ void umma_i8(unsigned tmem_d, unsigned long long adesc, unsigned long long bdesc, unsigned idesc,
                                        bool acc) {
  asm volatile("{\n.reg .pred p;\nsetp.ne.b32 p, %4, 0;\ntcgen05.mma.cta_group::1.kind::i8 [%0], %1, %2, %3, p;\n}\n" ::"r"(tmem_d),
               "l"(adesc), "l"(bdesc), "r"(idesc), "r"((int)acc));
}
__device__ __forceinline__ void umma_commit(unsigned long long* bar) {
  asm volatile("tcgen05.commit.cta_group::1.mbarrier::arrive::one.shared::cluster.b64 [%0];\n" ::"r"(smem_u32(bar)) : "memory");
}
__device__ __forceinline__ void tmem_ld8(unsigned taddr, int (&r)[8]) {
  asm volatile("tcgen05.ld.sync.aligned.32x32b.x8.b32 {%0,%1,%2,%3,%4,%5,%6,%7}, [%8];\n"
               : "=r"(r[0]), "=r"(r[1]), "=r"(r[2]), "=r"(r[3]), "=r"(r[4]), "=r"(r[5]), "=r"(r[6]), "=r"(r[7]) : "r"(taddr));
}

constexpr int GS_ROWS = 16, GS_CB = 4, GS_THREADS = 256, GS_TK = 512;
constexpr int GS_TKP = GS_TK + GS_TK / 8;
__device__ __forceinline__ int gs_tidx(int kk) { return kk + 2 * (kk >> 4); }

__device__ __forceinline__ void gs_roots(double (*sq)[GS_TKP], const double* __restrict__ S, int qp, int q, int ncb, int t0) {
  for (int id = threadIdx.x; id < GS_CB * GS_TK; id += GS_THREADS) {
    const int cb = id / GS_TK, kk = id % GS_TK, k = t0 + kk;
    sq[cb][gs_tidx(kk)] = cb < ncb && k < q ? sqrt(S[(size_t)cb * qp + k]) : 0.0;
  }
}

__device__ __forceinline__ void gs_load_x(double (&x)[16], const double* __restrict__ X, int np, int q, int row, int k0) {
  const bool full = k0 + 16 <= q;
#pragma unroll
  for (int j = 0; j < 16; ++j) x[j] = full || k0 + j < q ? X[row + (size_t)np * (k0 + j)] : 0.0;
}

__global__ void __launch_bounds__(GS_THREADS, 2) k_gram_slice(const double* __restrict__ X, const double* __restrict__ S,
                                                            int np, int q, int qp, int C, signed char* __restrict__ planes,
                                                            double* __restrict__ rscale) {
  __shared__ __align__(16) double sq[GS_CB][GS_TKP];
  __shared__ double red[GS_THREADS / 32][GS_CB][GS_ROWS];
  __shared__ double2 scl[GS_CB][GS_ROWS];
  const int lane = threadIdx.x & 31, warp = threadIdx.x >> 5, rr = lane & 15, h = lane >> 4;
  const int r0 = blockIdx.x * GS_ROWS, row = r0 + rr, c0 = blockIdx.y * GS_CB;
  const int ncb = C - c0 < GS_CB ? C - c0 : GS_CB;
  const double* Sb = S + (size_t)c0 * qp;
  constexpr int NW = GS_THREADS / 32, BPW = GS_TK / 32 / NW;
  double x[16];

  double m[GS_CB];
#pragma unroll
  for (int cb = 0; cb < GS_CB; ++cb) m[cb] = 0.0;
  for (int t0 = 0; t0 < q; t0 += GS_TK) {
    __syncthreads();
    gs_roots(sq, Sb, qp, q, ncb, t0);
    __syncthreads();
#pragma unroll
    for (int i = 0; i < BPW; ++i) {
      const int kk = 32 * (warp + NW * i) + 16 * h;
      if (t0 + kk >= q) continue;
      gs_load_x(x, X, np, q, row, t0 + kk);
#pragma unroll
      for (int cb = 0; cb < GS_CB; ++cb) {
        if (cb >= ncb) break;
#pragma unroll
        for (int j = 0; j < 16; j += 2) {
          const double2 s2 = *reinterpret_cast<const double2*>(&sq[cb][gs_tidx(kk + j)]);
          m[cb] = fmax(m[cb], fabs(x[j] * s2.x));
          m[cb] = fmax(m[cb], fabs(x[j + 1] * s2.y));
        }
      }
    }
  }
#pragma unroll
  for (int cb = 0; cb < GS_CB; ++cb) {
    const double o = __shfl_xor_sync(0xffffffffu, m[cb], 16);
    if (h == 0) red[warp][cb][rr] = fmax(m[cb], o);
  }
  __syncthreads();
  if (threadIdx.x < GS_CB * GS_ROWS) {
    const int cb = threadIdx.x / GS_ROWS, i = threadIdx.x % GS_ROWS;
    double mx = 0.0;
#pragma unroll
    for (int w = 0; w < NW; ++w) mx = fmax(mx, red[w][cb][i]);
    int p = 0;
    if (mx > 0.0) {
      p = 54 - ilogb(mx);
      if (ldexp(mx, p) > 126.0 * 0x1p48) --p;
    }
    if (cb < ncb) rscale[(size_t)(c0 + cb) * np + r0 + i] = ldexp(1.0, -p);
    const int p1 = p > 1000 ? 1000 : p;
    scl[cb][i] = make_double2(ldexp(1.0, p1), ldexp(1.0, p - p1));
  }

#if defined(GS_LAB_NO_STORES)
  unsigned sink = 0;
#endif
  for (int t0 = 0; t0 < qp; t0 += GS_TK) {
    __syncthreads();
    gs_roots(sq, Sb, qp, q, ncb, t0);
    __syncthreads();
#pragma unroll 1
    for (int i = 0; i < BPW; ++i) {
      const int kk = 32 * (warp + NW * i) + 16 * h;
      if (t0 + kk >= qp) continue;
      gs_load_x(x, X, np, q, row, t0 + kk);
#pragma unroll 1
      for (int cb = 0; cb < ncb; ++cb) {
        const double2 sc = scl[cb][rr];
        uint4 w[GI_S];
#pragma unroll
        for (int g = 0; g < 4; ++g) {
          unsigned lo[4], hi[4];
#pragma unroll
          for (int b = 0; b < 4; ++b) {
            const int j = 4 * g + b;
#if defined(GS_LAB_NO_DIGITS)
            lo[b] = __double2loint(x[j]) + j; hi[b] = __double2hiint(x[j]) + cb;
#else
            const double sqk = sq[cb][gs_tidx(kk + j)];
            const unsigned long long M = (unsigned long long)__double2ll_rn(x[j] * sqk * sc.x * sc.y) + 0x808080808080ull;
            lo[b] = (unsigned)M; hi[b] = (unsigned)(M >> 32);
#endif
          }
          const unsigned a0 = __byte_perm(lo[0], lo[1], 0x5140), a1 = __byte_perm(lo[0], lo[1], 0x7362);
          const unsigned a2 = __byte_perm(lo[2], lo[3], 0x5140), a3 = __byte_perm(lo[2], lo[3], 0x7362);
          const unsigned b0 = __byte_perm(hi[0], hi[1], 0x5140), b1 = __byte_perm(hi[0], hi[1], 0x7362);
          const unsigned b2 = __byte_perm(hi[2], hi[3], 0x5140), b3 = __byte_perm(hi[2], hi[3], 0x7362);
          const unsigned v[GI_S] = {__byte_perm(b1, b3, 0x5410), __byte_perm(b0, b2, 0x7632) ^ 0x80808080u,
                                    __byte_perm(b0, b2, 0x5410) ^ 0x80808080u, __byte_perm(a1, a3, 0x7632) ^ 0x80808080u,
                                    __byte_perm(a1, a3, 0x5410) ^ 0x80808080u, __byte_perm(a0, a2, 0x7632) ^ 0x80808080u,
                                    __byte_perm(a0, a2, 0x5410) ^ 0x80808080u};
#pragma unroll
          for (int s = 0; s < GI_S; ++s) (&w[s].x)[g] = v[s];
        }
        signed char* out = planes + ((size_t)(c0 + cb) * GI_S * np + row) * qp + t0 + kk;
#pragma unroll
        for (int s = 0; s < GI_S; ++s) {
#if defined(GS_LAB_NO_STORES)
          sink ^= w[s].x ^ w[s].y ^ w[s].z ^ w[s].w;
#else
          *reinterpret_cast<uint4*>(out + (size_t)s * np * qp) = w[s];
#endif
        }
      }
    }
  }
#if defined(GS_LAB_NO_STORES)
  if (sink == 0x9e3779b9u) planes[0] = 1;
#endif
}

__global__ void __launch_bounds__(GI_THREADS, 1)
k_gram_i8(const __grid_constant__ CUtensorMap tmA, const __grid_constant__ CUtensorMap tmB,
          const double* __restrict__ rscale, double* __restrict__ G, int np, int nvalid, int nkb) {
  extern __shared__ __align__(1024) unsigned char gsm_raw[];
  unsigned char* gsm = reinterpret_cast<unsigned char*>(((size_t)gsm_raw + 1023) & ~(size_t)1023);
  unsigned long long* full = reinterpret_cast<unsigned long long*>(gsm + (size_t)GI_STAGES * GI_STAGE_BYTES);
  unsigned long long* empty = full + GI_STAGES;
  unsigned long long* accf = empty + GI_STAGES;
  unsigned* tmem_slot = reinterpret_cast<unsigned*>(accf + 1);
  const int tid = threadIdx.x, lane = tid & 31, warp = tid >> 5;
  const int c = blockIdx.y;
  int ib = 0;
  while (2 * (ib + 1) * (ib + 2) / 2 <= (int)blockIdx.x) ++ib;
  const int jb = (int)blockIdx.x - ib * (ib + 1);
  const int i0 = ib * GI_BM, j0 = jb * GI_BN;
  const bool diag_block = (j0 / GI_BM) == ib;
  int rows_st = GI_BM;
  if (!diag_block) {
    int nfv = (nvalid - i0 + 7) / 8;
    if (nfv <= 0) return;
    rows_st = (nfv < 4 ? 4 : nfv) * 8;
  }
  if (tid == 0) {
    for (int s = 0; s < GI_STAGES; ++s) { mbar_init(&full[s], 1); mbar_init(&empty[s], 1); }
    mbar_init(accf, 1);
    asm volatile("fence.mbarrier_init.release.cluster;\n" ::: "memory");
  }
  if (warp == 0) {
    asm volatile("tcgen05.alloc.cta_group::1.sync.aligned.shared::cta.b32 [%0], 512;\n" ::"r"(smem_u32(tmem_slot)));
    asm volatile("tcgen05.relinquish_alloc_permit.cta_group::1.sync.aligned;\n");
  }
  asm volatile("tcgen05.fence::before_thread_sync;\n" ::: "memory");
  __syncthreads();
  asm volatile("tcgen05.fence::after_thread_sync;\n" ::: "memory");
  const unsigned tmem = *tmem_slot;

  if (warp == 4 && lane == 0) {
#if defined(GI_LAB_MMA_ONLY)
    for (int kb = 0; kb < GI_STAGES && kb < nkb; ++kb) {
#else
    for (int kb = 0; kb < nkb; ++kb) {
#endif
      const int st = kb % GI_STAGES;
      mbar_wait(&empty[st], ((kb / GI_STAGES) & 1) ^ 1);
      unsigned char* sa = gsm + (size_t)st * GI_STAGE_BYTES;
      mbar_expect_tx(&full[st], GI_STAGE_BYTES);
      tma_load_3d(sa, &tmA, kb * GI_BK, i0, c * GI_S, &full[st]);
      tma_load_3d(sa + GI_S * GI_A_PLANE, &tmB, kb * GI_BK, j0, c * GI_S, &full[st]);
    }
  } else if (warp == 5 && lane == 0) {
    for (int kb = 0; kb < nkb; ++kb) {
      const int st = kb % GI_STAGES;
#if defined(GI_LAB_MMA_ONLY)
      if (kb < GI_STAGES) mbar_wait(&full[st], 0);
#else
      mbar_wait(&full[st], (kb / GI_STAGES) & 1);
#endif
      asm volatile("tcgen05.fence::after_thread_sync;\n" ::: "memory");
#if defined(GI_LAB_LOADS_ONLY)
      umma_commit(&empty[st]);
      continue;
#endif
      const unsigned sa = smem_u32(gsm + (size_t)st * GI_STAGE_BYTES), sb = sa + GI_S * GI_A_PLANE;
#pragma unroll
      for (int kk = 0; kk < GI_BK / 32; ++kk) {
#pragma unroll
        for (int s = 0; s < GI_S; ++s) {
          const unsigned long long ad = gi_desc(sa + s * GI_A_PLANE + kk * 32);
#pragma unroll
          for (int t0 = 0; t0 < GI_S - s; t0 += 4) {
            const int nt = GI_S - s - t0 < 4 ? GI_S - s - t0 : 4;
            umma_i8(tmem + (unsigned)((s + t0) * GI_BN), ad, gi_desc(sb + t0 * GI_B_PLANE + kk * 32), gi_idesc(nt * GI_BN),
                    kb > 0 || kk > 0 || s > 0);
          }
        }
      }
      umma_commit(&empty[st]);
    }
    umma_commit(accf);
  } else if (warp < 4) {
    mbar_wait(accf, 0);
    asm volatile("tcgen05.fence::after_thread_sync;\n" ::: "memory");
    const int r = warp * 32 + lane, i = i0 + r;
    const double ri = rscale[(size_t)c * np + i] * 0x1p96;
    double* Gc = G + (size_t)c * np * np;
    const unsigned trow = tmem + ((unsigned)(warp * 32) << 16);
    for (int j8 = 0; j8 < GI_BN; j8 += 8) {
      int acc[GI_S][8];
#pragma unroll
      for (int g = 0; g < GI_S; ++g) tmem_ld8(trow + (unsigned)(g * GI_BN + j8), acc[g]);
      asm volatile("tcgen05.wait::ld.sync.aligned;\n" ::: "memory");
#pragma unroll
      for (int jj = 0; jj < 8; ++jj) {
        const int j = j0 + j8 + jj;
        double v = (double)acc[GI_S - 1][jj];
#pragma unroll
        for (int g = GI_S - 2; g >= 0; --g) v = (double)acc[g][jj] + v * 0x1p-8;
        v = v * ri * rscale[(size_t)c * np + j];
        if (i == j) v += 1.0;
        if (r < rows_st && (i >> 3) >= (j >> 3)) Gc[(size_t)j * np + i] = v;
      }
    }
  }
  asm volatile("tcgen05.fence::before_thread_sync;\n" ::: "memory");
  __syncthreads();
  if (warp == 0) {
    asm volatile("tcgen05.fence::after_thread_sync;\n" ::: "memory");
    asm volatile("tcgen05.dealloc.cta_group::1.sync.aligned.b32 %0, 512;\n" ::"r"(tmem));
  }
}

bool gram_i8_selected(const Dims& d) { return d.gmode == 1 && d.qp >= GRAM_I8_QP_MIN && d.qp <= GRAM_I8_QP_MAX; }

size_t gram_i8_plane_bytes(const Dims& d) { return (size_t)GI_S * d.np * d.qp; }

static CUresult encode_planes_map(CUtensorMap* m, const signed char* planes, const Dims& d, int C, uint32_t box_rows) {
  memset(m, 0, sizeof(*m));
  const cuuint64_t dims[3] = {(cuuint64_t)d.qp, (cuuint64_t)d.np, (cuuint64_t)GI_S * C};
  const cuuint64_t strides[2] = {(cuuint64_t)d.qp, (cuuint64_t)d.qp * d.np};
  const cuuint32_t box[3] = {(cuuint32_t)GI_BK, box_rows, (cuuint32_t)GI_S};
  const cuuint32_t estr[3] = {1, 1, 1};
  const CUtensorMapSwizzle sw = GI_BK == 128 ? CU_TENSOR_MAP_SWIZZLE_128B
                                             : (GI_BK == 64 ? CU_TENSOR_MAP_SWIZZLE_64B : CU_TENSOR_MAP_SWIZZLE_32B);
  if (!tmap_setup()) return CUDA_ERROR_NOT_SUPPORTED;
  return g_tmap_encode(m, CU_TENSOR_MAP_DATA_TYPE_UINT8, 3, const_cast<signed char*>(planes), dims, strides, box, estr,
                       CU_TENSOR_MAP_INTERLEAVE_NONE, sw, CU_TENSOR_MAP_L2_PROMOTION_L2_256B, CU_TENSOR_MAP_FLOAT_OOB_FILL_NONE);
}

static void launch_gram_i8_products(const Engine& e, cudaStream_t s) {
  const Dims& d = e.d;
  CUtensorMap tmA, tmB;
  if (encode_planes_map(&tmA, e.gram_planes, d, d.C, GI_BM) != CUDA_SUCCESS ||
      encode_planes_map(&tmB, e.gram_planes, d, d.C, GI_BN) != CUDA_SUCCESS) {
    fprintf(stderr, "[bnr] cuTensorMapEncodeTiled failed for the Gram digit planes (%d x %d)\n", d.np, d.qp);
    abort();
  }
  const int T = d.np / GI_BM;
  ++g_launches; k_gram_i8<<<dim3(T * (T + 1), d.C), GI_THREADS, GI_SMEM, s>>>(tmA, tmB, e.gram_rscale, e.G, d.np, d.n,
                                                                             (d.qp + GI_BK - 1) / GI_BK);
}

static void launch_gram_slice(const Engine& e, cudaStream_t s) {
  const Dims& d = e.d;
  ++g_launches; k_gram_slice<<<dim3(d.np / GS_ROWS, (d.C + GS_CB - 1) / GS_CB), GS_THREADS, 0, s>>>(
      e.X, e.S, d.np, d.q, d.qp, d.C, e.gram_planes, e.gram_rscale);
}

static void launch_gram_i8(const Engine& e, cudaStream_t s) {
  launch_gram_slice(e, s);
  launch_gram_i8_products(e, s);
}

void launch_syrk_G(const Engine& e, cudaStream_t s) {
  const Dims& d = e.d;
  if (gram_i8_selected(d)) {
    launch_gram_i8(e, s);
    if (e.aux.G_copy) {
      dim3 g2(d.np, d.C);
      ++g_launches; k_copy_sym<<<g2, 256, 0, s>>>(e.G, (size_t)d.np * d.np, d.np, e.aux.G_copy);
    }
    return;
  }
  const int T = d.np / SY_BT;
  const int nk = d.qp / SY_BK;
  const int ns = e.syrk_ws ? e.syrk_ws_cap + 1 : 1;
  const int nk_split = (nk + ns - 1) / ns;
#if defined(SYRK_LAB_ONLY_DIAG)
  dim3 grid(d.C, ns, T);
#elif defined(SYRK_LAB_ONLY_OFFDIAG)
  dim3 grid(d.C, ns, T * (T - 1) / 2);
#else
  dim3 grid(d.C, ns, T * (T + 1) / 2);
#endif
  const size_t gs = (size_t)d.np * d.np;
  const CUtensorMap tmX = make_map(e.X, d.np, d.qp, d.np, SY_LDS);
  ++g_launches; k_gram_syrk<<<grid, SY_THREADS, SYRK_SMEM, s>>>(tmX, e.S, (size_t)d.qp, e.G, gs, d.np, d.n, nk, 1.0,
                                                            nk_split, e.syrk_ws, e.syrk_ws_cap);
  if (ns > 1) {
    dim3 g2(T * (T + 1) / 2 * 8, d.C);
    ++g_launches; k_syrk_splitk_reduce<<<g2, 256, 0, s>>>(e.G, gs, d.np, e.syrk_ws, e.syrk_ws_cap, ns - 1);
  }
  if (e.aux.G_copy) {
    dim3 g2(d.np, d.C);
    ++g_launches; k_copy_sym<<<g2, 256, 0, s>>>(e.G, gs, d.np, e.aux.G_copy);
  }
}

void launch_xtx(const Dims& d, const double* XT, const double* ones, double* XtX, cudaStream_t s) {
  const int T = d.qp / SY_BT;
  dim3 grid(1, 1, T * (T + 1) / 2);
  const CUtensorMap tmXT = make_map(XT, d.qp, d.np, d.qp, SY_LDS);
  ++g_launches; k_gram_syrk<<<grid, SY_THREADS, SYRK_SMEM, s>>>(tmXT, ones, 0, XtX, 0, d.qp, d.q, d.np / SY_BK, 0.0,
                                                            d.np / SY_BK, nullptr, 0);
}

__global__ void __launch_bounds__(256) k_build_P(Engine e) {
  const Dims& d = e.d;
  if (blockIdx.x < blockIdx.y) return;
  const int c = blockIdx.z, N = d.qp;
  const int i = blockIdx.x * 32 + threadIdx.x;
  const double it2 = 1.0 / e.tau2[c];
  double* Gc = e.G + (size_t)c * N * N;
#pragma unroll
  for (int jj = 0; jj < 4; ++jj) {
    const int j = blockIdx.y * 32 + threadIdx.y * 4 + jj;
    if (i < j) continue;
    double v;
    if (i < d.q) {
      v = e.XtX[(size_t)j * N + i] * it2;
      if (i == j) v = (e.XtX[(size_t)j * N + i] + 1.0 / e.S[(size_t)c * d.qp + j]) * it2;
    } else {
      v = (i == j) ? 1.0 : 0.0;
    }
    Gc[(size_t)j * N + i] = v;
  }
}

void launch_build_P(const Engine& e, cudaStream_t s) {
  const Dims& d = e.d;
  dim3 grid(d.qp / 32, d.qp / 32, d.C), block(32, 8);
  ++g_launches; k_build_P<<<grid, block, 0, s>>>(e);
  if (e.aux.G_copy) {
    dim3 g2(d.qp, d.C);
    ++g_launches; k_copy_sym<<<g2, 256, 0, s>>>(e.G, (size_t)d.qp * d.qp, d.qp, e.aux.G_copy);
  }
}

void launch_cholesky(const Engine& e, double* rhs, const ForkJoin& fj, cudaStream_t s) {
  const Dims& d = e.d;
  const int N = d.gdim;
  const int m = d.gmode == 2 ? d.q : d.n;
  const size_t cs = (size_t)N * N;
  const int T = N / PB;
  const size_t ls = (size_t)T * PB * PB;
  const bool latency = (long long)d.C_total * (T - 1) <= 128;
  ++g_launches; k_augment<<<d.C, 256, 0, s>>>(e.G, cs, N, m, rhs, d.gmode == 2 ? d.qp : d.np, d.gmode == 2 ? e.S : nullptr, e.tau2);
  const CUtensorMap mG = make_map(e.G, N, (uint64_t)N * d.C, N, SY_LDS);
  const CUtensorMap mG2 = make_map(e.G, N, (uint64_t)N * d.C, N, SY_BT / 2 + 4);
  const CUtensorMap mG4 = make_map(e.G, N, (uint64_t)N * d.C, N, SY_BT / 4 + 4);
  const CUtensorMap mL = make_map(e.Linv, PB, (uint64_t)PB * T * d.C, PB, SY_LDS);
  auto mI = [&](int ns) -> const CUtensorMap& { return ns == 4 ? mG4 : (ns == 2 ? mG2 : mG); };

  if (!latency) {
    cudaStream_t sideA = fj.side_hi;
    for (int J = 0; J < T; ++J) {
      const bool fork = J > 0 && J + 1 < T;
      if (J > 0) {
        const int nk = J * PB / SY_BK;
        if (fork) {
          cudaEventRecord(fj.fork, s);
          cudaStreamWaitEvent(sideA, fj.fork, 0);
          dim3 g2(d.C, T - J - 1);
          ++g_launches; k_chol_update<<<g2, SY_THREADS, SYRK_SMEM, sideA>>>(mG, mG, 0, e.G, cs, N, m + 1, nk, J, J + 1, 1);
          cudaEventRecord(fj.join, sideA);
          dim3 g1(d.C, 1);
          ++g_launches; k_chol_update<<<g1, SY_THREADS, SYRK_SMEM, s>>>(mG, mG, 0, e.G, cs, N, m + 1, nk, J, J, 1);
        } else {
          dim3 g2(d.C, T - J);
          ++g_launches; k_chol_update<<<g2, SY_THREADS, SYRK_SMEM, s>>>(mG, mG, 0, e.G, cs, N, m + 1, nk, J, J, 1);
        }
      }
      ++g_launches; k_potf2_inv<<<d.C, 256, POTF2_SMEM, s>>>(e.G, cs, N, J, e.Linv, T, e.status, 0);
      if (fork) cudaStreamWaitEvent(s, fj.join, 0);
      if (J + 1 < T) {
        dim3 g1(d.C, T - J - 1);
        ++g_launches; k_trsm_dmma<<<g1, SY_THREADS, SYRK_SMEM, s>>>(mL, mG, e.G, cs, N, m + 1, J, J + 1, 1);
      }
    }
    return;
  }

  cudaStream_t side = fj.side_hi;
  cudaEvent_t* evP = fj.pool;
  cudaEvent_t* evT = fj.pool + T;
  cudaEvent_t* evL = fj.pool + 2 * T;
  cudaEvent_t* evE = fj.pool + 3 * T;
  auto strips = [&](int tiles) {
    const int ctas = d.C_total * tiles;
    return ctas * 4 <= 148 ? 4 : (ctas * 2 <= 148 ? 2 : 1);
  };
  auto launch_trsm = [&](int J, int ib_first, int rows, int ns, cudaStream_t st) {
    dim3 g(d.C, rows * ns);
    const double* Lj = e.Linv + (size_t)J * PB * PB;
    ++g_launches;
    if (ns == 8)
      k_small_tile<2, 2><<<g, 256, small_tile_smem(16), st>>>(e.G, cs, N, J, ib_first, 8, Lj, ls, PB, J * PB, 0);
    else if (ns == 4)
      k_small_tile<2, 4><<<g, 256, small_tile_smem(32), st>>>(e.G, cs, N, J, ib_first, 4, Lj, ls, PB, J * PB, 0);
    else if (ns == 2)
      k_small_tile<2, 8><<<g, 256, small_tile_smem(64), st>>>(e.G, cs, N, J, ib_first, 2, Lj, ls, PB, J * PB, 0);
    else
      k_trsm_dmma<<<g, SY_THREADS, SYRK_SMEM, st>>>(mL, mG, e.G, cs, N, m + 1, J, ib_first, 1);
  };
  const bool quiet = d.gmode == 2 || e.syrk_ws != nullptr;
  const int ud = quiet ? (d.C_total * 8 <= 148 ? 8 : (d.C_total * 4 <= 148 ? 4 : 0)) : 0;
  for (int J = 0; J < T; ++J) {
    const bool has_side = J + 2 < T;
    if (J >= 2 && !ud) cudaStreamWaitEvent(s, evE[J - 2], 0);
    ++g_launches; k_potf2_inv<<<d.C, 256, POTF2_SMEM, s>>>(e.G, cs, N, J, e.Linv, T, e.status, (J > 0 && !ud) ? 1 : 0);
    if (has_side) cudaEventRecord(evP[J], s);
    if (J + 1 < T) {
      if (J >= 1) cudaStreamWaitEvent(s, evL[J - 1], 0);
      const int ns1 = ud ? ud : strips(1);
      launch_trsm(J, J + 1, 1, ns1, s);
      if (has_side) cudaEventRecord(evT[J], s);
      if (ud) {
        if (J >= 1) cudaStreamWaitEvent(s, evE[J - 1], 0);
        dim3 gd(d.C, ud);
        const double* Lt = e.G + (size_t)J * PB * N + (size_t)(J + 1) * PB;
        ++g_launches;
        if (ud == 8) k_small_tile<1, 2><<<gd, 256, small_tile_smem(16), s>>>(e.G, cs, N, J + 1, J + 1, 8, Lt, cs, N, J * PB, 1);
        else k_small_tile<1, 4><<<gd, 256, small_tile_smem(32), s>>>(e.G, cs, N, J + 1, J + 1, 4, Lt, cs, N, J * PB, 1);
      }
    }
    if (has_side) {
      const int rows = T - J - 2;
      cudaStreamWaitEvent(side, evP[J], 0);
      const int ns2 = strips(rows);
      dim3 g2(d.C, rows * ns2);
      launch_trsm(J, J + 2, rows, ns2, side);
      cudaStreamWaitEvent(side, evT[J], 0);
      ++g_launches;
      if (ns2 == 4)
        k_small_tile<1, 4><<<g2, 256, small_tile_smem(32), side>>>(e.G, cs, N, J + 1, J + 2, 4, e.G + (size_t)J * PB * N + (size_t)(J + 1) * PB, cs, N, J * PB, 0);
      else if (ns2 == 2)
        k_small_tile<1, 8><<<g2, 256, small_tile_smem(64), side>>>(e.G, cs, N, J + 1, J + 2, 2, e.G + (size_t)J * PB * N + (size_t)(J + 1) * PB, cs, N, J * PB, 0);
      else
        k_chol_update<<<g2, SY_THREADS, SYRK_SMEM, side>>>(mG, mG, J * PB, e.G, cs, N, m + 1, PB / SY_BK, J + 1, J + 2, 1);
      cudaEventRecord(evL[J], side);
      ++g_launches; k_chol_update<<<g2, SY_THREADS, SYRK_SMEM, side>>>(mG, mI(ns2), 0, e.G, cs, N, m + 1, (J + 1) * PB / SY_BK,
                                                                   J + 2, J + 2, ns2);
      cudaEventRecord(evE[J], side);
    }
  }
}

void launch_chol_solve(const Engine& e, double* out, const double* addz, cudaStream_t s) {
  const Dims& d = e.d;
  const int N = d.gdim;
  const int m = d.gmode == 2 ? d.q : d.n;
  const int stride = d.gmode == 2 ? d.qp : d.np;
  const CUtensorMap tmG = make_map(e.G, N, (uint64_t)N * d.C, N, PB, BW_COLS);
  const CUtensorMap tmL = make_map(e.Linv, PB, (uint64_t)PB * (N / PB) * d.C, PB, PB, BW_COLS);
  if (N <= BWD_STREAM_MAX_DIM) {
    ++g_launches; k_bwd_stream<<<d.C, BW_THREADS, bwd_smem(N), s>>>(tmG, tmL, e.G, (size_t)N * N, N, m, out, stride, addz,
                                                                 stride, bwd_stages(N));
    return;
  }
  cudaLaunchConfig_t cfg = {};
  cudaLaunchAttribute attr[1];
  attr[0].id = cudaLaunchAttributeClusterDimension;
  attr[0].val.clusterDim.x = BWC_K; attr[0].val.clusterDim.y = 1; attr[0].val.clusterDim.z = 1;
  cfg.gridDim = dim3(d.C * BWC_K);
  cfg.blockDim = dim3(BW_THREADS);
  cfg.dynamicSmemBytes = bwc_smem(N);
  cfg.stream = s;
  cfg.attrs = attr;
  cfg.numAttrs = 1;
  ++g_launches;
  cudaLaunchKernelEx(&cfg, k_bwd_cluster, tmG, tmL, (const double*)e.G, (size_t)N * N, N, m, out, stride, addz, stride,
                     bwc_stages(N));
}

int bwd_cluster_capacity(int N) {
  if (N <= BWD_STREAM_MAX_DIM) return 1;
  cudaLaunchConfig_t cfg = {};
  cudaLaunchAttribute attr[1];
  attr[0].id = cudaLaunchAttributeClusterDimension;
  attr[0].val.clusterDim.x = BWC_K; attr[0].val.clusterDim.y = 1; attr[0].val.clusterDim.z = 1;
  cfg.gridDim = dim3(BWC_K);
  cfg.blockDim = dim3(BW_THREADS);
  cfg.dynamicSmemBytes = bwc_smem(N);
  cfg.attrs = attr;
  cfg.numAttrs = 1;
  int n = 0;
  if (cudaOccupancyMaxActiveClusters(&n, k_bwd_cluster, &cfg) != cudaSuccess) return -1;
  return n;
}

int chol_max_dim() { return CHOL_MAX_DIM; }
int bwd_stream_max_dim() { return BWD_STREAM_MAX_DIM; }

}
```

Before: 11780.

## Fuse Gram digit slicing into persistent int8 Gram kernel with ring buffer

```diff
diff --git a/bayesiannetworkregression.jl_b200/csrc/bnr_api.cu b/bayesiannetworkregression.jl_b200/csrc/bnr_api.cu
--- a/bayesiannetworkregression.jl_b200/csrc/bnr_api.cu
+++ b/bayesiannetworkregression.jl_b200/csrc/bnr_api.cu
@@ -346,9 +346,8 @@
   DA(e.Linv, C * (size_t)(d.gdim / TILE_N) * TILE_N * TILE_N);
   CK(cudaMemsetAsync(e.Linv, 0, sizeof(double) * C * (size_t)(d.gdim / TILE_N) * TILE_N * TILE_N, h->stream));
   e.syrk_ws = nullptr; e.syrk_ws_cap = 0;
-  e.gram_planes = nullptr; e.gram_rscale = nullptr;
+  e.gram_planes = nullptr; e.gram_rscale = nullptr; e.gram_state = nullptr;
   if (gram_i8_selected(d)) {
-    DA(e.gram_planes, C * gram_i8_plane_bytes(d));
     DA(e.gram_rscale, C * d.np);
   } else if (d.gmode == BNR_GAMMA_NFORM) {
     const int smax = syrk_splits(d, d.C);
@@ -405,6 +404,10 @@
     if (ng > MAX_GROUPS) ng = MAX_GROUPS;
     if (ng > d.C) ng = d.C;
     h->n_groups = ng;
+    if (gram_i8_selected(d)) {
+      DA(e.gram_planes, (size_t)ng * gram_i8_ring_chains(d) * gram_i8_plane_bytes(d));
+      DA(e.gram_state, (size_t)ng * gram_i8_state_words(d));
+    }
     CK(cudaEventCreateWithFlags(&h->ev_fork, cudaEventDisableTiming));
     const int panels = d.gdim / TILE_N;
     if (int r = create_fork_join(h->fj, panels, 0, 0)) return r;
@@ -580,7 +583,7 @@
   mark(marks, 8, s);
 }
 
-static Engine group_view(const bnr_handle* h, int c0, int Cg, long long* counters, long long* mom_window) {
+static Engine group_view(const bnr_handle* h, int g, int c0, int Cg, long long* counters, long long* mom_window) {
   Engine v = h->e;
   const Dims& d = h->e.d;
   const size_t c = (size_t)c0;
@@ -593,7 +596,11 @@
   v.M += c * d.R * d.R; v.lambda += c * d.R; v.pi += c * 3 * d.R;
   v.xg += c * d.np; v.xv += c * d.np; v.rhs += c * d.np;
   v.G += c * d.gdim * d.gdim; if (v.syrk_ws) v.syrk_ws += c * (size_t)v.syrk_ws_cap * d.gdim * d.gdim; v.Linv += c * (size_t)(d.gdim / TILE_N) * TILE_N * TILE_N;
-  if (v.gram_planes) { v.gram_planes += c * gram_i8_plane_bytes(d); v.gram_rscale += c * d.np; }
+  if (v.gram_planes) {
+    v.gram_planes += (size_t)g * gram_i8_ring_chains(d) * gram_i8_plane_bytes(d);
+    v.gram_state += (size_t)g * gram_i8_state_words(d);
+    v.gram_rscale += c * d.np;
+  }
   v.partials += c * d.nparts * (2 * MAX_R + 1);
   v.moments += c * 2 * (d.V + d.q) * 2;
   if (v.bmom) v.bmom += c * (size_t)v.bmom_nb * (d.V + d.q) * 2;
@@ -621,7 +628,7 @@
     ChainGroup& G = h->groups[g];
     const int c0 = (int)((long long)C * g / ng), c1 = (int)((long long)C * (g + 1) / ng);
     G.c0 = c0;
-    G.e = group_view(h, c0, c1 - c0, G.counters, G.mom_window);
+    G.e = group_view(h, g, c0, c1 - c0, G.counters, G.mom_window);
     Engine e = G.e;
     CK(cudaStreamBeginCapture(G.stream, cudaStreamCaptureModeThreadLocal));
     enqueue_sweep(e, G.ws, G.fj, G.stream);
diff --git a/bayesiannetworkregression.jl_b200/csrc/bnr_engine.cuh b/bayesiannetworkregression.jl_b200/csrc/bnr_engine.cuh
--- a/bayesiannetworkregression.jl_b200/csrc/bnr_engine.cuh
+++ b/bayesiannetworkregression.jl_b200/csrc/bnr_engine.cuh
@@ -115,6 +115,7 @@
   int syrk_ws_cap;
   signed char* gram_planes;
   double* gram_rscale;
+  unsigned* gram_state;
   double* Linv;
   double* partials;
   double* tau2_part;
diff --git a/bayesiannetworkregression.jl_b200/csrc/bnr_kernels.h b/bayesiannetworkregression.jl_b200/csrc/bnr_kernels.h
--- a/bayesiannetworkregression.jl_b200/csrc/bnr_kernels.h
+++ b/bayesiannetworkregression.jl_b200/csrc/bnr_kernels.h
@@ -48,6 +48,8 @@
 constexpr int GRAM_I8_QP_MAX = 18724;
 bool gram_i8_selected(const Dims& d);
 size_t gram_i8_plane_bytes(const Dims& d);
+int gram_i8_ring_chains(const Dims& d);
+size_t gram_i8_state_words(const Dims& d);
 struct ForkJoin {
   cudaStream_t side = nullptr;
   cudaStream_t side_hi = nullptr;
diff --git a/bayesiannetworkregression.jl_b200/csrc/bnr_linalg.cu b/bayesiannetworkregression.jl_b200/csrc/bnr_linalg.cu
--- a/bayesiannetworkregression.jl_b200/csrc/bnr_linalg.cu
+++ b/bayesiannetworkregression.jl_b200/csrc/bnr_linalg.cu
@@ -1396,7 +1396,9 @@
 }
 
 __global__ void k_gram_i8(const __grid_constant__ CUtensorMap tmA, const __grid_constant__ CUtensorMap tmB,
-                          const double* __restrict__ rscale, double* __restrict__ G, int np, int nvalid, int nkb);
+                          const double* __restrict__ X, const double* __restrict__ S, double* rscale,
+                          double* __restrict__ G, signed char* planes, unsigned* state, int np, int nvalid, int q, int qp,
+                          int C, int ring, int nkb);
 extern const size_t GI_SMEM_BYTES;
 
 void linalg_setup() {
@@ -1489,9 +1491,6 @@
 constexpr int GI_STAGES = BNR_GI_STAGES;
 constexpr int GI_A_PLANE = GI_BM * GI_BK, GI_B_PLANE = GI_BN * GI_BK;
 constexpr int GI_STAGE_BYTES = GI_S * (GI_A_PLANE + GI_B_PLANE);
-constexpr size_t GI_SMEM = (size_t)GI_STAGES * GI_STAGE_BYTES + 1024 + 256;
-const size_t GI_SMEM_BYTES = GI_SMEM;
-constexpr int GI_THREADS = 192;
 static_assert(GI_BK == 32 || GI_BK == 64 || GI_BK == 128, "k-block = swizzle width");
 static_assert(GI_S * GI_BN <= 512, "accumulators exceed tensor memory");
 
@@ -1521,12 +1520,26 @@
                : "=r"(r[0]), "=r"(r[1]), "=r"(r[2]), "=r"(r[3]), "=r"(r[4]), "=r"(r[5]), "=r"(r[6]), "=r"(r[7]) : "r"(taddr));
 }
 
-constexpr int GS_ROWS = 16, GS_CB = 4, GS_THREADS = 256, GS_TK = 512;
+constexpr int GS_ROWS = 16, GS_CB = 4, GS_THREADS = 128, GS_TK = 512;
 constexpr int GS_TKP = GS_TK + GS_TK / 8;
+constexpr int GS_NW = GS_THREADS / 32;
+struct GsScratch {
+  double sq[GS_CB][GS_TKP];
+  double red[GS_NW][GS_CB][GS_ROWS];
+  double2 scl[GS_CB][GS_ROWS];
+};
+constexpr int GI_THREADS = 320;
+constexpr size_t GI_SMEM = (size_t)GI_STAGES * GI_STAGE_BYTES + 2 * sizeof(GsScratch) + 1024 + 256;
+const size_t GI_SMEM_BYTES = GI_SMEM;
+static_assert(GI_SMEM <= 227 * 1024, "k_gram_i8 exceeds the shared memory of a CTA");
 __device__ __forceinline__ int gs_tidx(int kk) { return kk + 2 * (kk >> 4); }
-
-__device__ __forceinline__ void gs_roots(double (*sq)[GS_TKP], const double* __restrict__ S, int qp, int q, int ncb, int t0) {
-  for (int id = threadIdx.x; id < GS_CB * GS_TK; id += GS_THREADS) {
+__device__ __forceinline__ void bar_named(int id, int threads) {
+  asm volatile("bar.sync %0, %1;\n" ::"r"(id), "r"(threads) : "memory");
+}
+
+__device__ __forceinline__ void gs_roots(double (*sq)[GS_TKP], const double* __restrict__ S, int qp, int q, int ncb, int t0,
+                                         int lt) {
+  for (int id = lt; id < GS_CB * GS_TK; id += GS_THREADS) {
     const int cb = id / GS_TK, kk = id % GS_TK, k = t0 + kk;
     sq[cb][gs_tidx(kk)] = cb < ncb && k < q ? sqrt(S[(size_t)cb * qp + k]) : 0.0;
   }
@@ -1538,29 +1551,22 @@
   for (int j = 0; j < 16; ++j) x[j] = full || k0 + j < q ? X[row + (size_t)np * (k0 + j)] : 0.0;
 }
 
-__global__ void __launch_bounds__(GS_THREADS, 2) k_gram_slice(const double* __restrict__ X, const double* __restrict__ S,
-                                                            int np, int q, int qp, int C, signed char* __restrict__ planes,
-                                                            double* __restrict__ rscale) {
-  __shared__ __align__(16) double sq[GS_CB][GS_TKP];
-  __shared__ double red[GS_THREADS / 32][GS_CB][GS_ROWS];
-  __shared__ double2 scl[GS_CB][GS_ROWS];
-  const int lane = threadIdx.x & 31, warp = threadIdx.x >> 5, rr = lane & 15, h = lane >> 4;
-  const int r0 = blockIdx.x * GS_ROWS, row = r0 + rr, c0 = blockIdx.y * GS_CB;
-  const int ncb = C - c0 < GS_CB ? C - c0 : GS_CB;
-  const double* Sb = S + (size_t)c0 * qp;
-  constexpr int NW = GS_THREADS / 32, BPW = GS_TK / 32 / NW;
+__device__ void gs_slab(GsScratch& sm, int bar, int lt, const double* __restrict__ X, const double* __restrict__ S, int np,
+                        int q, int qp, int ncb, int r0, signed char* __restrict__ pl, double* __restrict__ rs) {
+  const int lane = lt & 31, warp = lt >> 5, rr = lane & 15, h = lane >> 4, row = r0 + rr;
+  constexpr int BPW = GS_TK / 32 / GS_NW;
   double x[16];
 
   double m[GS_CB];
 #pragma unroll
   for (int cb = 0; cb < GS_CB; ++cb) m[cb] = 0.0;
   for (int t0 = 0; t0 < q; t0 += GS_TK) {
-    __syncthreads();
-    gs_roots(sq, Sb, qp, q, ncb, t0);
-    __syncthreads();
+    bar_named(bar, GS_THREADS);
+    gs_roots(sm.sq, S, qp, q, ncb, t0, lt);
+    bar_named(bar, GS_THREADS);
 #pragma unroll
     for (int i = 0; i < BPW; ++i) {
-      const int kk = 32 * (warp + NW * i) + 16 * h;
+      const int kk = 32 * (warp + GS_NW * i) + 16 * h;
       if (t0 + kk >= q) continue;
       gs_load_x(x, X, np, q, row, t0 + kk);
 #pragma unroll
@@ -1568,7 +1574,7 @@
         if (cb >= ncb) break;
 #pragma unroll
         for (int j = 0; j < 16; j += 2) {
-          const double2 s2 = *reinterpret_cast<const double2*>(&sq[cb][gs_tidx(kk + j)]);
+          const double2 s2 = *reinterpret_cast<const double2*>(&sm.sq[cb][gs_tidx(kk + j)]);
           m[cb] = fmax(m[cb], fabs(x[j] * s2.x));
           m[cb] = fmax(m[cb], fabs(x[j + 1] * s2.y));
         }
@@ -1578,39 +1584,36 @@
 #pragma unroll
   for (int cb = 0; cb < GS_CB; ++cb) {
     const double o = __shfl_xor_sync(0xffffffffu, m[cb], 16);
-    if (h == 0) red[warp][cb][rr] = fmax(m[cb], o);
-  }
-  __syncthreads();
-  if (threadIdx.x < GS_CB * GS_ROWS) {
-    const int cb = threadIdx.x / GS_ROWS, i = threadIdx.x % GS_ROWS;
+    if (h == 0) sm.red[warp][cb][rr] = fmax(m[cb], o);
+  }
+  bar_named(bar, GS_THREADS);
+  if (lt < GS_CB * GS_ROWS) {
+    const int cb = lt / GS_ROWS, i = lt % GS_ROWS;
     double mx = 0.0;
 #pragma unroll
-    for (int w = 0; w < NW; ++w) mx = fmax(mx, red[w][cb][i]);
+    for (int w = 0; w < GS_NW; ++w) mx = fmax(mx, sm.red[w][cb][i]);
     int p = 0;
     if (mx > 0.0) {
       p = 54 - ilogb(mx);
       if (ldexp(mx, p) > 126.0 * 0x1p48) --p;
     }
-    if (cb < ncb) rscale[(size_t)(c0 + cb) * np + r0 + i] = ldexp(1.0, -p);
+    if (cb < ncb) rs[(size_t)cb * np + r0 + i] = ldexp(1.0, -p);
     const int p1 = p > 1000 ? 1000 : p;
-    scl[cb][i] = make_double2(ldexp(1.0, p1), ldexp(1.0, p - p1));
-  }
-
-#if defined(GS_LAB_NO_STORES)
-  unsigned sink = 0;
-#endif
+    sm.scl[cb][i] = make_double2(ldexp(1.0, p1), ldexp(1.0, p - p1));
+  }
+
   for (int t0 = 0; t0 < qp; t0 += GS_TK) {
-    __syncthreads();
-    gs_roots(sq, Sb, qp, q, ncb, t0);
-    __syncthreads();
+    bar_named(bar, GS_THREADS);
+    gs_roots(sm.sq, S, qp, q, ncb, t0, lt);
+    bar_named(bar, GS_THREADS);
 #pragma unroll 1
     for (int i = 0; i < BPW; ++i) {
-      const int kk = 32 * (warp + NW * i) + 16 * h;
+      const int kk = 32 * (warp + GS_NW * i) + 16 * h;
       if (t0 + kk >= qp) continue;
       gs_load_x(x, X, np, q, row, t0 + kk);
 #pragma unroll 1
       for (int cb = 0; cb < ncb; ++cb) {
-        const double2 sc = scl[cb][rr];
+        const double2 sc = sm.scl[cb][rr];
         uint4 w[GI_S];
 #pragma unroll
         for (int g = 0; g < 4; ++g) {
@@ -1618,13 +1621,9 @@
 #pragma unroll
           for (int b = 0; b < 4; ++b) {
             const int j = 4 * g + b;
-#if defined(GS_LAB_NO_DIGITS)
-            lo[b] = __double2loint(x[j]) + j; hi[b] = __double2hiint(x[j]) + cb;
-#else
-            const double sqk = sq[cb][gs_tidx(kk + j)];
+            const double sqk = sm.sq[cb][gs_tidx(kk + j)];
             const unsigned long long M = (unsigned long long)__double2ll_rn(x[j] * sqk * sc.x * sc.y) + 0x808080808080ull;
             lo[b] = (unsigned)M; hi[b] = (unsigned)(M >> 32);
-#endif
           }
           const unsigned a0 = __byte_perm(lo[0], lo[1], 0x5140), a1 = __byte_perm(lo[0], lo[1], 0x7362);
           const unsigned a2 = __byte_perm(lo[2], lo[3], 0x5140), a3 = __byte_perm(lo[2], lo[3], 0x7362);
@@ -1637,48 +1636,95 @@
 #pragma unroll
           for (int s = 0; s < GI_S; ++s) (&w[s].x)[g] = v[s];
         }
-        signed char* out = planes + ((size_t)(c0 + cb) * GI_S * np + row) * qp + t0 + kk;
-#pragma unroll
-        for (int s = 0; s < GI_S; ++s) {
-#if defined(GS_LAB_NO_STORES)
-          sink ^= w[s].x ^ w[s].y ^ w[s].z ^ w[s].w;
-#else
-          *reinterpret_cast<uint4*>(out + (size_t)s * np * qp) = w[s];
+        signed char* out = pl + ((size_t)cb * GI_S * np + row) * qp + t0 + kk;
+#pragma unroll
+        for (int s = 0; s < GI_S; ++s) *reinterpret_cast<uint4*>(out + (size_t)s * np * qp) = w[s];
+      }
+    }
+  }
+  asm volatile("fence.proxy.async.global;\n" ::: "memory");
+  bar_named(bar, GS_THREADS);
+}
+
+__device__ __forceinline__ unsigned ld_acquire(const unsigned* p) {
+  unsigned v;
+  asm volatile("ld.acquire.gpu.global.u32 %0, [%1];\n" : "=r"(v) : "l"(p) : "memory");
+  return v;
+}
+__device__ __forceinline__ void st_release(unsigned* p, unsigned v) {
+  asm volatile("st.release.gpu.global.u32 [%0], %1;\n" ::"l"(p), "r"(v) : "memory");
+}
+__device__ __forceinline__ void red_release_add(unsigned* p, unsigned v) {
+  asm volatile("red.release.gpu.global.add.u32 [%0], %1;\n" ::"l"(p), "r"(v) : "memory");
+}
+__device__ __forceinline__ unsigned ld_volatile(const unsigned* p) { return *(const volatile unsigned*)p; }
+
+struct GiTile { int c, i0, j0, rows_st; bool diag; };
+__device__ __forceinline__ GiTile gi_tile(unsigned t, int tpc, int nvalid) {
+  GiTile r;
+  r.c = (int)(t / (unsigned)tpc);
+  const int x = (int)(t % (unsigned)tpc);
+  int ib = 0;
+  while ((ib + 1) * (ib + 2) <= x) ++ib;
+  r.i0 = ib * GI_BM; r.j0 = (x - ib * (ib + 1)) * GI_BN;
+  r.diag = (r.j0 / GI_BM) == ib;
+  r.rows_st = GI_BM;
+  if (!r.diag) {
+    const int nfv = (nvalid - r.i0 + 7) / 8;
+    r.rows_st = nfv <= 0 ? 0 : (nfv < 4 ? 4 : nfv) * 8;
+  }
+  return r;
+}
+
+struct GiState {
+  unsigned *tile, *done, *next, *ready;
+  int C, nb, nslab, tpc, rb;
+  __device__ GiState(unsigned* st, int C_, int np, int tpc_, int ring)
+      : C(C_), nb((C_ + GS_CB - 1) / GS_CB), nslab(np / GS_ROWS), tpc(tpc_), rb((ring + GS_CB - 1) / GS_CB) {
+    tile = st; done = st + 1; next = done + nb; ready = next + nb;
+  }
+  __device__ bool slot_free(int b) const {
+    if (b < rb) return true;
+    const int pb = b - rb, nch = C - GS_CB * pb < GS_CB ? C - GS_CB * pb : GS_CB;
+    return ld_acquire(done + pb) == (unsigned)(nch * tpc);
+  }
+};
+
+__device__ __forceinline__ void gi_slice(GsScratch& sm, int bar, int lt, const GiState& st, int b, int s,
+                                         const double* __restrict__ X, const double* __restrict__ S, int np, int q, int qp,
+                                         int ring, signed char* planes, double* rscale) {
+  const int c0 = b * GS_CB, ncb = st.C - c0 < GS_CB ? st.C - c0 : GS_CB;
+  gs_slab(sm, bar, lt, X, S + (size_t)c0 * qp, np, q, qp, ncb, s * GS_ROWS,
+          planes + (size_t)(c0 % ring) * GI_S * np * qp, rscale + (size_t)c0 * np);
+  if (lt == 0) { __threadfence(); st_release(st.ready + (size_t)b * st.nslab + s, 1u); }
+}
+
+#if defined(DIAG_PROF)
+__device__ unsigned long long g_diag[8];
 #endif
-        }
-      }
-    }
-  }
-#if defined(GS_LAB_NO_STORES)
-  if (sink == 0x9e3779b9u) planes[0] = 1;
-#endif
-}
-
 __global__ void __launch_bounds__(GI_THREADS, 1)
-k_gram_i8(const __grid_constant__ CUtensorMap tmA, const __grid_constant__ CUtensorMap tmB,
-          const double* __restrict__ rscale, double* __restrict__ G, int np, int nvalid, int nkb) {
+k_gram_i8(const __grid_constant__ CUtensorMap tmA, const __grid_constant__ CUtensorMap tmB, const double* __restrict__ X,
+          const double* __restrict__ S, double* rscale, double* __restrict__ G, signed char* planes, unsigned* state, int np,
+          int nvalid, int q, int qp, int C, int ring, int nkb) {
   extern __shared__ __align__(1024) unsigned char gsm_raw[];
   unsigned char* gsm = reinterpret_cast<unsigned char*>(((size_t)gsm_raw + 1023) & ~(size_t)1023);
-  unsigned long long* full = reinterpret_cast<unsigned long long*>(gsm + (size_t)GI_STAGES * GI_STAGE_BYTES);
+  GsScratch* scr = reinterpret_cast<GsScratch*>(gsm + (size_t)GI_STAGES * GI_STAGE_BYTES);
+  unsigned long long* full = reinterpret_cast<unsigned long long*>(scr + 2);
   unsigned long long* empty = full + GI_STAGES;
   unsigned long long* accf = empty + GI_STAGES;
   unsigned* tmem_slot = reinterpret_cast<unsigned*>(accf + 1);
+  volatile unsigned* sm_tile = tmem_slot + 1;
+  volatile int* sm_over = reinterpret_cast<volatile int*>(tmem_slot + 2);
+  volatile int* sm_act = sm_over + 1;
+  volatile int* sm_pact = sm_over + 2;
   const int tid = threadIdx.x, lane = tid & 31, warp = tid >> 5;
-  const int c = blockIdx.y;
-  int ib = 0;
-  while (2 * (ib + 1) * (ib + 2) / 2 <= (int)blockIdx.x) ++ib;
-  const int jb = (int)blockIdx.x - ib * (ib + 1);
-  const int i0 = ib * GI_BM, j0 = jb * GI_BN;
-  const bool diag_block = (j0 / GI_BM) == ib;
-  int rows_st = GI_BM;
-  if (!diag_block) {
-    int nfv = (nvalid - i0 + 7) / 8;
-    if (nfv <= 0) return;
-    rows_st = (nfv < 4 ? 4 : nfv) * 8;
-  }
+  const int T = np / GI_BM, tpc = T * (T + 1);
+  const unsigned total = (unsigned)tpc * C;
+  const GiState st(state, C, np, tpc, ring);
   if (tid == 0) {
     for (int s = 0; s < GI_STAGES; ++s) { mbar_init(&full[s], 1); mbar_init(&empty[s], 1); }
     mbar_init(accf, 1);
+    *sm_over = 0;
     asm volatile("fence.mbarrier_init.release.cluster;\n" ::: "memory");
   }
   if (warp == 0) {
@@ -1690,71 +1736,187 @@
   asm volatile("tcgen05.fence::after_thread_sync;\n" ::: "memory");
   const unsigned tmem = *tmem_slot;
 
-  if (warp == 4 && lane == 0) {
-#if defined(GI_LAB_MMA_ONLY)
-    for (int kb = 0; kb < GI_STAGES && kb < nkb; ++kb) {
-#else
-    for (int kb = 0; kb < nkb; ++kb) {
+  if (warp >= 4 && warp < 8) {
+    const int lt = tid - 128;
+    int pb = 0;
+    for (;;) {
+      if (lt == 0) {
+        int act = -2;
+        while (pb < st.nb && ld_volatile(st.next + pb) >= (unsigned)st.nslab) ++pb;
+        if (pb < st.nb && !*sm_over) {
+          act = -1;
+          for (int b = pb; b < st.nb && b < pb + st.rb; ++b) {
+            if (ld_volatile(st.next + b) >= (unsigned)st.nslab) continue;
+            if (!st.slot_free(b)) break;
+            const unsigned s = atomicAdd(st.next + b, 1u);
+            if (s < (unsigned)st.nslab) { act = b * st.nslab + (int)s; break; }
+          }
+          if (act == -1) __nanosleep(2000);
+        }
+        *sm_pact = act;
+      }
+      bar_named(2, GS_THREADS);
+      const int act = *sm_pact;
+      bar_named(2, GS_THREADS);
+      if (act == -2) break;
+      if (act >= 0) gi_slice(scr[1], 2, lt, st, act / st.nslab, act % st.nslab, X, S, np, q, qp, ring, planes, rscale);
+#if defined(DIAG_PROF)
+      if (act >= 0 && lt == 0) atomicAdd(&g_diag[4], 1ull);
 #endif
-      const int st = kb % GI_STAGES;
-      mbar_wait(&empty[st], ((kb / GI_STAGES) & 1) ^ 1);
-      unsigned char* sa = gsm + (size_t)st * GI_STAGE_BYTES;
-      mbar_expect_tx(&full[st], GI_STAGE_BYTES);
-      tma_load_3d(sa, &tmA, kb * GI_BK, i0, c * GI_S, &full[st]);
-      tma_load_3d(sa + GI_S * GI_A_PLANE, &tmB, kb * GI_BK, j0, c * GI_S, &full[st]);
-    }
-  } else if (warp == 5 && lane == 0) {
-    for (int kb = 0; kb < nkb; ++kb) {
-      const int st = kb % GI_STAGES;
-#if defined(GI_LAB_MMA_ONLY)
-      if (kb < GI_STAGES) mbar_wait(&full[st], 0);
-#else
-      mbar_wait(&full[st], (kb / GI_STAGES) & 1);
+    }
+  } else {
+    constexpr int TB = 192;
+    for (int it = 0;; ++it) {
+      if (tid == 0) {
+        unsigned t;
+        for (;;) {
+#if defined(DIAG_TILES_PER_CTA)
+          if (it >= DIAG_TILES_PER_CTA) { t = total; *sm_over = 1; break; }
 #endif
+          t = atomicAdd(st.tile, 1u);
+          if (t >= total) { *sm_over = 1; break; }
+          const GiTile tl = gi_tile(t, tpc, nvalid);
+          if (tl.rows_st > 0) break;
+          red_release_add(st.done + tl.c / GS_CB, 1u);
+        }
+        *sm_tile = t;
+      }
+      bar_named(3, TB);
+      const unsigned t = *sm_tile;
+      if (t >= total) break;
+      const GiTile tl = gi_tile(t, tpc, nvalid);
+      const int c = tl.c, b = c / GS_CB, i0 = tl.i0, j0 = tl.j0;
+#if defined(DIAG_PROF)
+      long long tc0 = clock64();
+#endif
+      if (warp < 4) {
+        const int sa = i0 / GS_ROWS, sb = j0 / GS_ROWS;
+        const int last = sa + GI_BM / GS_ROWS - 1 > sb + GI_BN / GS_ROWS - 1 ? sa + GI_BM / GS_ROWS - 1 : sb + GI_BN / GS_ROWS - 1;
+        for (;;) {
+          if (tid == 0) {
+            int act = -1;
+            if (ld_volatile(st.next + b) <= (unsigned)last) {
+              while (!st.slot_free(b)) __nanosleep(256);
+              const unsigned s = atomicAdd(st.next + b, 1u);
+              if (s < (unsigned)st.nslab) act = (int)s;
+            }
+            *sm_act = act;
+          }
+          bar_named(1, GS_THREADS);
+          const int act = *sm_act;
+          bar_named(1, GS_THREADS);
+          if (act < 0) break;
+          gi_slice(scr[0], 1, tid, st, b, act, X, S, np, q, qp, ring, planes, rscale);
+#if defined(DIAG_PROF)
+          if (tid == 0) atomicAdd(&g_diag[2], 1ull);
+#endif
+        }
+        if (tid == 0) {
+          const unsigned* rd = st.ready + (size_t)b * st.nslab;
+          for (int s = sa; s < sa + GI_BM / GS_ROWS; ++s) while (!ld_acquire(rd + s)) __nanosleep(128);
+          for (int s = sb; s < sb + GI_BN / GS_ROWS; ++s) while (!ld_acquire(rd + s)) __nanosleep(128);
+        }
+      }
+      bar_named(3, TB);
+#if defined(DIAG_PROF)
+      if (tid == 0) { atomicAdd(&g_diag[0], (unsigned long long)(clock64() - tc0)); atomicAdd(&g_diag[3], 1ull); }
+#endif
+      const int z = (c % ring) * GI_S;
+      if (warp == 8) {
+        if (lane == 0) {
+          asm volatile("fence.proxy.async.global;\n" ::: "memory");
+          for (int kb = 0; kb < nkb; ++kb) {
+            const int g = it * nkb + kb, sg = g % GI_STAGES;
+            mbar_wait(&empty[sg], ((g / GI_STAGES) & 1) ^ 1);
+            unsigned char* sa = gsm + (size_t)sg * GI_STAGE_BYTES;
+            mbar_expect_tx(&full[sg], GI_STAGE_BYTES);
+            tma_load_3d(sa, &tmA, kb * GI_BK, i0, z, &full[sg]);
+            tma_load_3d(sa + GI_S * GI_A_PLANE, &tmB, kb * GI_BK, j0, z, &full[sg]);
+          }
+        }
+      } else if (warp == 9) {
+        if (lane == 0) {
+          for (int kb = 0; kb < nkb; ++kb) {
+            const int g = it * nkb + kb, sg = g % GI_STAGES;
+            mbar_wait(&full[sg], (g / GI_STAGES) & 1);
+            asm volatile("tcgen05.fence::after_thread_sync;\n" ::: "memory");
+            const unsigned sa = smem_u32(gsm + (size_t)sg * GI_STAGE_BYTES), sb = sa + GI_S * GI_A_PLANE;
+#pragma unroll
+            for (int kk = 0; kk < GI_BK / 32; ++kk) {
+#pragma unroll
+              for (int s = 0; s < GI_S; ++s) {
+                const unsigned long long ad = gi_desc(sa + s * GI_A_PLANE + kk * 32);
+#pragma unroll
+                for (int t0 = 0; t0 < GI_S - s; t0 += 4) {
+                  const int nt = GI_S - s - t0 < 4 ? GI_S - s - t0 : 4;
+                  umma_i8(tmem + (unsigned)((s + t0) * GI_BN), ad, gi_desc(sb + t0 * GI_B_PLANE + kk * 32),
+                          gi_idesc(nt * GI_BN), kb > 0 || kk > 0 || s > 0);
+                }
+              }
+            }
+            umma_commit(&empty[sg]);
+          }
+          umma_commit(accf);
+        }
+      } else {
+#if defined(DIAG_EPI_SLICE)
+        for (;;) {
+          if (tid == 0) {
+            int act = -1;
+            unsigned ok;
+            asm volatile("{\n.reg .pred p;\nmbarrier.test_wait.parity.shared::cta.b64 p, [%1], %2;\nselp.u32 %0, 1, 0, p;\n}\n"
+                         : "=r"(ok) : "r"(smem_u32(accf)), "r"((unsigned)(it & 1)) : "memory");
+            if (!ok) {
+              for (int bb = b; bb < st.nb && bb < b + st.rb; ++bb) {
+                if (ld_volatile(st.next + bb) >= (unsigned)st.nslab) continue;
+                if (!st.slot_free(bb)) break;
+                const unsigned s = atomicAdd(st.next + bb, 1u);
+                if (s < (unsigned)st.nslab) { act = bb * st.nslab + (int)s; break; }
+              }
+            }
+            *sm_act = act;
+          }
+          bar_named(1, GS_THREADS);
+          const int act = *sm_act;
+          bar_named(1, GS_THREADS);
+          if (act < 0) break;
+          gi_slice(scr[0], 1, tid, st, act / st.nslab, act % st.nslab, X, S, np, q, qp, ring, planes, rscale);
+        }
+#endif
+#if defined(DIAG_PROF)
+        long long tw0 = clock64();
+#endif
+        mbar_wait(accf, it & 1);
+#if defined(DIAG_PROF)
+        if (tid == 0) atomicAdd(&g_diag[1], (unsigned long long)(clock64() - tw0));
+#endif
+        asm volatile("tcgen05.fence::after_thread_sync;\n" ::: "memory");
+        const int r = warp * 32 + lane, i = i0 + r;
+        const double* rsc = rscale + (size_t)c * np;
+        const double ri = __ldcg(rsc + i) * 0x1p96;
+        double* Gc = G + (size_t)c * np * np;
+        const unsigned trow = tmem + ((unsigned)(warp * 32) << 16);
+        for (int j8 = 0; j8 < GI_BN; j8 += 8) {
+          int acc[GI_S][8];
+#pragma unroll
+          for (int g = 0; g < GI_S; ++g) tmem_ld8(trow + (unsigned)(g * GI_BN + j8), acc[g]);
+          asm volatile("tcgen05.wait::ld.sync.aligned;\n" ::: "memory");
+#pragma unroll
+          for (int jj = 0; jj < 8; ++jj) {
+            const int j = j0 + j8 + jj;
+            double v = (double)acc[GI_S - 1][jj];
+#pragma unroll
+            for (int g = GI_S - 2; g >= 0; --g) v = (double)acc[g][jj] + v * 0x1p-8;
+            v = v * ri * __ldcg(rsc + j);
+            if (i == j) v += 1.0;
+            if (r < tl.rows_st && (i >> 3) >= (j >> 3)) Gc[(size_t)j * np + i] = v;
+          }
+        }
+      }
+      asm volatile("tcgen05.fence::before_thread_sync;\n" ::: "memory");
+      bar_named(3, TB);
       asm volatile("tcgen05.fence::after_thread_sync;\n" ::: "memory");
-#if defined(GI_LAB_LOADS_ONLY)
-      umma_commit(&empty[st]);
-      continue;
-#endif
-      const unsigned sa = smem_u32(gsm + (size_t)st * GI_STAGE_BYTES), sb = sa + GI_S * GI_A_PLANE;
-#pragma unroll
-      for (int kk = 0; kk < GI_BK / 32; ++kk) {
-#pragma unroll
-        for (int s = 0; s < GI_S; ++s) {
-          const unsigned long long ad = gi_desc(sa + s * GI_A_PLANE + kk * 32);
-#pragma unroll
-          for (int t0 = 0; t0 < GI_S - s; t0 += 4) {
-            const int nt = GI_S - s - t0 < 4 ? GI_S - s - t0 : 4;
-            umma_i8(tmem + (unsigned)((s + t0) * GI_BN), ad, gi_desc(sb + t0 * GI_B_PLANE + kk * 32), gi_idesc(nt * GI_BN),
-                    kb > 0 || kk > 0 || s > 0);
-          }
-        }
-      }
-      umma_commit(&empty[st]);
-    }
-    umma_commit(accf);
-  } else if (warp < 4) {
-    mbar_wait(accf, 0);
-    asm volatile("tcgen05.fence::after_thread_sync;\n" ::: "memory");
-    const int r = warp * 32 + lane, i = i0 + r;
-    const double ri = rscale[(size_t)c * np + i] * 0x1p96;
-    double* Gc = G + (size_t)c * np * np;
-    const unsigned trow = tmem + ((unsigned)(warp * 32) << 16);
-    for (int j8 = 0; j8 < GI_BN; j8 += 8) {
-      int acc[GI_S][8];
-#pragma unroll
-      for (int g = 0; g < GI_S; ++g) tmem_ld8(trow + (unsigned)(g * GI_BN + j8), acc[g]);
-      asm volatile("tcgen05.wait::ld.sync.aligned;\n" ::: "memory");
-#pragma unroll
-      for (int jj = 0; jj < 8; ++jj) {
-        const int j = j0 + j8 + jj;
-        double v = (double)acc[GI_S - 1][jj];
-#pragma unroll
-        for (int g = GI_S - 2; g >= 0; --g) v = (double)acc[g][jj] + v * 0x1p-8;
-        v = v * ri * rscale[(size_t)c * np + j];
-        if (i == j) v += 1.0;
-        if (r < rows_st && (i >> 3) >= (j >> 3)) Gc[(size_t)j * np + i] = v;
-      }
+      if (tid == 0) red_release_add(st.done + b, 1u);
     }
   }
   asm volatile("tcgen05.fence::before_thread_sync;\n" ::: "memory");
@@ -1769,9 +1931,28 @@
 
 size_t gram_i8_plane_bytes(const Dims& d) { return (size_t)GI_S * d.np * d.qp; }
 
-static CUresult encode_planes_map(CUtensorMap* m, const signed char* planes, const Dims& d, int C, uint32_t box_rows) {
+#ifndef DIAG_RING_EXTRA
+#define DIAG_RING_EXTRA 2
+#endif
+int gram_i8_ring_chains(const Dims& d) {
+  int dev = 0, sms = 0;
+  cudaGetDevice(&dev);
+  cudaDeviceGetAttribute(&sms, cudaDevAttrMultiProcessorCount, dev);
+  const int T = d.np / GI_BM, block_tiles = GS_CB * T * (T + 1);
+  int blocks = (sms + block_tiles - 1) / block_tiles + DIAG_RING_EXTRA;
+  if (blocks < 3) blocks = 3;
+  return d.C_total < blocks * GS_CB ? d.C_total : blocks * GS_CB;
+}
+
+static size_t gram_i8_state_words(const Dims& d, int C) {
+  const size_t nb = (size_t)(C + GS_CB - 1) / GS_CB;
+  return 1 + 2 * nb + nb * (size_t)(d.np / GS_ROWS);
+}
+size_t gram_i8_state_words(const Dims& d) { return gram_i8_state_words(d, d.C_total); }
+
+static CUresult encode_planes_map(CUtensorMap* m, const signed char* planes, const Dims& d, int ring, uint32_t box_rows) {
   memset(m, 0, sizeof(*m));
-  const cuuint64_t dims[3] = {(cuuint64_t)d.qp, (cuuint64_t)d.np, (cuuint64_t)GI_S * C};
+  const cuuint64_t dims[3] = {(cuuint64_t)d.qp, (cuuint64_t)d.np, (cuuint64_t)GI_S * ring};
   const cuuint64_t strides[2] = {(cuuint64_t)d.qp, (cuuint64_t)d.qp * d.np};
   const cuuint32_t box[3] = {(cuuint32_t)GI_BK, box_rows, (cuuint32_t)GI_S};
   const cuuint32_t estr[3] = {1, 1, 1};
@@ -1782,28 +1963,29 @@
                        CU_TENSOR_MAP_INTERLEAVE_NONE, sw, CU_TENSOR_MAP_L2_PROMOTION_L2_256B, CU_TENSOR_MAP_FLOAT_OOB_FILL_NONE);
 }
 
-static void launch_gram_i8_products(const Engine& e, cudaStream_t s) {
+static void launch_gram_i8(const Engine& e, cudaStream_t s) {
   const Dims& d = e.d;
+  const int ring = gram_i8_ring_chains(d);
   CUtensorMap tmA, tmB;
-  if (encode_planes_map(&tmA, e.gram_planes, d, d.C, GI_BM) != CUDA_SUCCESS ||
-      encode_planes_map(&tmB, e.gram_planes, d, d.C, GI_BN) != CUDA_SUCCESS) {
+  if (encode_planes_map(&tmA, e.gram_planes, d, ring, GI_BM) != CUDA_SUCCESS ||
+      encode_planes_map(&tmB, e.gram_planes, d, ring, GI_BN) != CUDA_SUCCESS) {
     fprintf(stderr, "[bnr] cuTensorMapEncodeTiled failed for the Gram digit planes (%d x %d)\n", d.np, d.qp);
     abort();
   }
-  const int T = d.np / GI_BM;
-  ++g_launches; k_gram_i8<<<dim3(T * (T + 1), d.C), GI_THREADS, GI_SMEM, s>>>(tmA, tmB, e.gram_rscale, e.G, d.np, d.n,
-                                                                             (d.qp + GI_BK - 1) / GI_BK);
-}
-
-static void launch_gram_slice(const Engine& e, cudaStream_t s) {
-  const Dims& d = e.d;
-  ++g_launches; k_gram_slice<<<dim3(d.np / GS_ROWS, (d.C + GS_CB - 1) / GS_CB), GS_THREADS, 0, s>>>(
-      e.X, e.S, d.np, d.q, d.qp, d.C, e.gram_planes, e.gram_rscale);
-}
-
-static void launch_gram_i8(const Engine& e, cudaStream_t s) {
-  launch_gram_slice(e, s);
-  launch_gram_i8_products(e, s);
+  int dev = 0, sms = 0;
+  cudaGetDevice(&dev);
+  cudaDeviceGetAttribute(&sms, cudaDevAttrMultiProcessorCount, dev);
+  const int T = d.np / GI_BM, tiles = T * (T + 1) * d.C;
+  ++g_launches; cudaMemsetAsync(e.gram_state, 0, sizeof(unsigned) * gram_i8_state_words(d, d.C), s);
+  int grid = tiles < sms ? tiles : sms;
+#if defined(DIAG_TILES_PER_CTA)
+  grid = (tiles + DIAG_TILES_PER_CTA - 1) / DIAG_TILES_PER_CTA;
+#elif defined(DIAG_GRID_SHARE)
+  grid = (sms * d.C + d.C_total - 1) / d.C_total; if (grid > tiles) grid = tiles;
+#endif
+  ++g_launches; k_gram_i8<<<grid, GI_THREADS, GI_SMEM, s>>>(
+      tmA, tmB, e.X, e.S, e.gram_rscale, e.G, e.gram_planes, e.gram_state, d.np, d.n, d.q, d.qp, d.C, ring,
+      (d.qp + GI_BK - 1) / GI_BK);
 }
 
 void launch_syrk_G(const Engine& e, cudaStream_t s) {
```

Result: slower. 9817 (median of 6 runs) (-16.7%).
